# prismformore/Multi-Task-Transformer

Measured on NVIDIA H100. Metric: images/sec, higher is better.
Workload: dtype bf16x3 (split-bf16 operands, fp32 accumulate)

## Files before the change

### multi-task-transformer_b200/csrc/gemm_common.cuh

```cuda
#pragma once
#include "host_common.h"
#include "ptx.cuh"

namespace mtt {

constexpr int BM = 128;
constexpr int BK = 64;
constexpr int kEpiWarps = 8;
constexpr int kGemmThreads = 128 + kEpiWarps * 32;
constexpr uint32_t kTileBytes = BM * BK * 2;

struct GemmParams {
  int M, N;
  int num_kb, taps, ksize, dil, mode;
  int NB, H, W, TW, TH, tiles_x, tiles_y;
  int tiles_m;
  int tiles_n;
  int cin_pad;
  int k_last_steps;
  uint32_t a_box_bytes;
  const float* bias;
  int act;
  const float* residual;
  long long ldr;
  int res_row_mod;
  float* out_f32;
  long long ldo_f32;
  __nv_bfloat16* out_hi;
  __nv_bfloat16* out_lo;
  long long ldo_bf;
  int in_group, out_group, out_offset;
  int out_row_stride;
  int vec_ok;
  int a_groups_per_tile;
  int debug;
  int sk_tiles;
  float* sk_part;
  unsigned int* sk_flags;
};

constexpr size_t kSkFlagBytes = 16384;
constexpr size_t sk_workspace_bytes(int units) { return kSkFlagBytes + (size_t)units * BM * 256 * 4; }

constexpr int kMaxGroup = 32;
struct GroupProblem {
  const float* bias;
  const float* residual;
  float* out_f32;
  __nv_bfloat16* out_hi;
  __nv_bfloat16* out_lo;
};
struct GemmGroup {
  int count;
  int tiles_per_problem;
  GroupProblem prob[kMaxGroup];
};
struct GemmGroupMaps {
  CUtensorMap m[kMaxGroup][4];
};

int gemm_prepare(const mtt_gemm_desc* d, int b_box_rows, GemmParams& p, CUtensorMap maps[4]);

template <int NSPLIT>
__device__ __forceinline__ void load_a_tile(const GemmParams& p, const CUtensorMap* tmA_hi,
                                            const CUtensorMap* tmA_lo, uint8_t* sa, uint64_t* bar, int ms,
                                            int kb, int dy, int dx) {
  auto ld2 = [&](void* dst, const CUtensorMap* m, int c0, int c1) { tma_load_2d(dst, m, bar, c0, c1); };
  auto ld3 = [&](void* dst, const CUtensorMap* m, int c0, int c1, int c2) { tma_load_3d(dst, m, bar, c0, c1, c2); };
  auto ld4 = [&](void* dst, const CUtensorMap* m, int c0, int c1, int c2, int c3) {
    tma_load_4d(dst, m, bar, c0, c1, c2, c3);
  };
  if (p.mode == 0 && p.a_groups_per_tile > 0) {
    ld3(sa, tmA_hi, kb * BK, 0, ms * p.a_groups_per_tile);
    if (NSPLIT == 2) ld3(sa + kTileBytes, tmA_lo, kb * BK, 0, ms * p.a_groups_per_tile);
  } else if (p.mode == 0) {
    ld2(sa, tmA_hi, kb * BK, ms * BM);
    if (NSPLIT == 2) ld2(sa + kTileBytes, tmA_lo, kb * BK, ms * BM);
  } else {
    const int per_img = p.tiles_x * p.tiles_y;
    const int cb = ms / per_img;
    const int r = ms - cb * per_img;
    const int cy = (r / p.tiles_x) * p.TH + dy;
    const int cx = (r % p.tiles_x) * p.TW + dx;
    ld4(sa, tmA_hi, kb * BK, cx, cy, cb);
    if (NSPLIT == 2) ld4(sa + kTileBytes, tmA_lo, kb * BK, cx, cy, cb);
  }
}

struct RowInfo {
  long long mo;
  long long mr;
  bool ok;
};
__device__ __forceinline__ RowInfo row_info(const GemmParams& p, int ms, int row) {
  RowInfo r;
  long long m;
  if (p.mode == 0) {
    m = (long long)ms * BM + row;
    r.ok = m < p.M;
    if (p.a_groups_per_tile > 0) r.ok = r.ok && ms < p.tiles_m;
  } else {
    const int per_img = p.tiles_x * p.tiles_y;
    const int cb = ms / per_img;
    const int t = ms - cb * per_img;
    const int y = (t / p.tiles_x) * p.TH + row / p.TW;
    const int x = (t % p.tiles_x) * p.TW + row % p.TW;
    r.ok = (cb < p.NB) && (row < p.TW * p.TH) && (y < p.H) && (x < p.W);
    m = ((long long)cb * p.H + y) * p.W + x;
  }
  r.mo = m;
  if (p.in_group > 0) r.mo = (m / p.in_group) * p.out_group + p.out_offset + (m % p.in_group) * p.out_row_stride;
  r.mr = (p.res_row_mod > 0) ? (m % p.res_row_mod) : r.mo;
  return r;
}

enum { kOutF32 = 1, kOutSplit = 2, kOutBoth = 3 };

__device__ __forceinline__ float4 epilogue_bias4(const GemmParams& p, int n, bool full) {
  float4 b = make_float4(0.f, 0.f, 0.f, 0.f);
  if (!p.bias) return b;
  if (full) return __ldg(reinterpret_cast<const float4*>(p.bias + n));
  if (n < p.N) b.x = __ldg(p.bias + n);
  if (n + 1 < p.N) b.y = __ldg(p.bias + n + 1);
  if (n + 2 < p.N) b.z = __ldg(p.bias + n + 2);
  if (n + 3 < p.N) b.w = __ldg(p.bias + n + 3);
  return b;
}
template <int ACT>
__device__ __forceinline__ float epilogue_op(float v, float b, float r, bool bias, bool res) {
  if (bias) v += b;
  if (ACT == MTT_ACT_GELU) v = gelu_erf(v);
  if (ACT == MTT_ACT_RELU) v = fmaxf(v, 0.f);
  if (res) v += r;
  return v;
}
template <int ACT, int OUT>
__device__ __forceinline__ void epilogue_store4(const GemmParams& p, float4 v, float4 b, float4 r, long long of,
                                                long long ob, int n, bool full) {
  const bool bias = p.bias != nullptr, res = p.residual != nullptr;
  v.x = epilogue_op<ACT>(v.x, b.x, r.x, bias, res);
  v.y = epilogue_op<ACT>(v.y, b.y, r.y, bias, res);
  v.z = epilogue_op<ACT>(v.z, b.z, r.z, bias, res);
  v.w = epilogue_op<ACT>(v.w, b.w, r.w, bias, res);
  if (p.debug & 4) {
    asm volatile("" ::"f"(v.x), "f"(v.y), "f"(v.z), "f"(v.w));
    return;
  }
  if (full) {
    if (OUT & kOutF32) *reinterpret_cast<float4*>(p.out_f32 + of) = v;
    if (OUT & kOutSplit) {
      uint2 h, l;
      split_pack2(v.x, v.y, h.x, l.x);
      split_pack2(v.z, v.w, h.y, l.y);
      *reinterpret_cast<uint2*>(p.out_hi + ob) = h;
      if (p.out_lo) *reinterpret_cast<uint2*>(p.out_lo + ob) = l;
    }
    return;
  }
  const float e[4] = {v.x, v.y, v.z, v.w};
#pragma unroll
  for (int k = 0; k < 4; ++k) {
    if (n + k >= p.N) break;
    if (OUT & kOutF32) p.out_f32[of + k] = e[k];
    if (OUT & kOutSplit) {
      __nv_bfloat16 h, l;
      split_bf16(e[k], h, l);
      p.out_hi[ob + k] = h;
      if (p.out_lo) p.out_lo[ob + k] = l;
    }
  }
}

int launch_gemm_tiles(const mtt_gemm_desc* d, int bn, cudaStream_t stream);
int launch_gemm_tiles_grouped(const mtt_gemm_desc* d, int count, int bn, cudaStream_t stream);
void set_gemm_streamk(int mode);
int streamk_tiles(int tiles, int k_iters, int pairs);
int streamk_schedule_host(int tiles, int k_iters, int pairs, int pair, int* out, int max_pieces);

}
```

### multi-task-transformer_b200/csrc/gemm_host.cu

```cuda
#include <stdlib.h>

#include "gemm_common.cuh"

namespace mtt {

static void pick_conv_tile(int H, int W, int* TW, int* TH) {
  double best = -1;
  int btw = 1, bth = 1;
  for (int tw = 1; tw <= 128 && tw <= W; ++tw) {
    int th = 128 / tw;
    if (th > H) th = H;
    if (th < 1) continue;
    const long long tiles = (long long)((W + tw - 1) / tw) * ((H + th - 1) / th);
    const double eff = (double)H * W / ((double)tiles * 128.0);
    if (eff > best + 1e-9 || (eff > best - 1e-9 && tw > btw)) {
      best = eff;
      btw = tw;
      bth = th;
    }
  }
  *TW = btw;
  *TH = bth;
}

static int make_split_maps(const void* hi, const void* lo, int nsplit, int rank, const uint64_t* dims,
                           const uint64_t* strides, const uint32_t* box, CUtensorMap* maps) {
  int rc = make_tmap_bf16(&maps[0], hi, rank, dims, strides, box);
  if (rc) return rc;
  if (nsplit == 2) return make_tmap_bf16(&maps[1], lo, rank, dims, strides, box);
  maps[1] = maps[0];
  return MTT_OK;
}

int gemm_prepare(const mtt_gemm_desc* d, int b_box_rows, GemmParams& p, CUtensorMap maps[4]) {
  if (!d) return set_error(MTT_ERR_BAD_SHAPE, "mtt_gemm: null descriptor");
  if (d->M <= 0 || d->N <= 0 || d->K <= 0)
    return set_error(MTT_ERR_BAD_SHAPE, "mtt_gemm: M=%d N=%d K=%d must be positive", d->M, d->N, d->K);
  if (d->nsplit != 1 && d->nsplit != 2)
    return set_error(MTT_ERR_BAD_SHAPE, "mtt_gemm: nsplit=%d (1 or 2)", d->nsplit);
  if (!d->a_hi || !d->b_hi || (d->nsplit == 2 && (!d->a_lo || !d->b_lo)))
    return set_error(MTT_ERR_BAD_SHAPE, "mtt_gemm: missing operand plane");
  if (!d->out_f32 && !d->out_hi) return set_error(MTT_ERR_BAD_SHAPE, "mtt_gemm: no output");
  if (d->act != MTT_ACT_NONE && d->act != MTT_ACT_GELU && d->act != MTT_ACT_RELU)
    return set_error(MTT_ERR_BAD_SHAPE, "mtt_gemm: act=%d (0 none, 1 GELU, 2 ReLU)", d->act);
  if (d->lda % 8 || d->ldb % 8)
    return set_error(MTT_ERR_MISALIGNED, "mtt_gemm: lda=%lld ldb=%lld must be multiples of 8",
                     (long long)d->lda, (long long)d->ldb);

  p = GemmParams{};
  {
    static int dbg = -1;
    if (dbg < 0) {
      const char* e = getenv("MTT_GEMM_DEBUG");
      dbg = e ? atoi(e) : 0;
    }
    p.debug = dbg;
  }
  p.M = d->M;
  p.N = d->N;
  p.mode = d->mode;
  p.num_kb = (d->K + BK - 1) / BK;
  p.k_last_steps = (d->K - (p.num_kb - 1) * BK + 15) / 16;
  p.tiles_n = 0;
  p.bias = d->bias;
  p.act = d->act;
  p.residual = d->residual;
  p.ldr = d->ldr;
  p.res_row_mod = d->res_row_mod;
  p.out_f32 = d->out_f32;
  p.ldo_f32 = d->ldo_f32;
  p.out_hi = static_cast<__nv_bfloat16*>(d->out_hi);
  p.out_lo = static_cast<__nv_bfloat16*>(d->out_lo);
  p.ldo_bf = d->ldo_bf;
  p.in_group = d->in_group;
  p.out_group = d->out_group;
  p.out_offset = d->out_offset;
  p.out_row_stride = d->out_row_stride > 1 ? d->out_row_stride : 1;
  if (p.out_hi && d->nsplit == 2 && !p.out_lo)
    return set_error(MTT_ERR_BAD_SHAPE, "mtt_gemm: out_lo missing for nsplit=2");

  auto al16 = [](const void* q) { return (reinterpret_cast<uintptr_t>(q) & 15) == 0; };
  p.vec_ok = 1;
  if (d->bias && !al16(d->bias)) p.vec_ok = 0;
  if (d->residual && (!al16(d->residual) || d->ldr % 4)) p.vec_ok = 0;
  if (d->out_f32 && (!al16(d->out_f32) || d->ldo_f32 % 4)) p.vec_ok = 0;
  if (d->out_hi && (!al16(d->out_hi) || d->ldo_bf % 8 || (p.out_lo && !al16(p.out_lo)))) p.vec_ok = 0;

  int rc;
  const int ksq = (d->mode == 1) ? d->ksize * d->ksize : 1;
  if (d->mode == 0 && d->a_group_rows > 0) {
    const int g = d->a_group_rows;
    if (g > BM || d->M % g || d->a_group_stride < g)
      return set_error(MTT_ERR_BAD_SHAPE, "mtt_gemm: a_group_rows=%d must divide M=%d and be <= %d", g, d->M, BM);
    const int ngroups = d->M / g;
    const int gpt = BM / g;
    if (ngroups > gpt && BM % g)
      return set_error(MTT_ERR_BAD_SHAPE, "mtt_gemm: %d groups of %d rows need %d %% %d == 0", ngroups, g, BM, g);
    p.taps = 1;
    p.ksize = 1;
    p.dil = 1;
    p.cin_pad = 0;
    p.a_groups_per_tile = ngroups < gpt ? ngroups : gpt;
    p.tiles_m = (ngroups + p.a_groups_per_tile - 1) / p.a_groups_per_tile;
    if (p.tiles_m > 1 && p.a_groups_per_tile * g != BM)
      return set_error(MTT_ERR_BAD_SHAPE, "mtt_gemm: gathered A tiles must be full");
    p.a_box_bytes = (uint32_t)(p.a_groups_per_tile * g) * BK * 2;
    const uint64_t dims[3] = {(uint64_t)d->K, (uint64_t)g, (uint64_t)ngroups};
    const uint64_t str[2] = {(uint64_t)d->lda * 2, (uint64_t)d->a_group_stride * d->lda * 2};
    const uint32_t box[3] = {BK, (uint32_t)g, (uint32_t)p.a_groups_per_tile};
    if ((rc = make_split_maps(d->a_hi, d->a_lo, d->nsplit, 3, dims, str, box, &maps[0]))) return rc;
  } else if (d->mode == 0) {
    p.taps = 1;
    p.ksize = 1;
    p.dil = 1;
    p.cin_pad = 0;
    p.tiles_m = (d->M + BM - 1) / BM;
    p.a_box_bytes = kTileBytes;
    const uint64_t dims[2] = {(uint64_t)d->K, (uint64_t)d->M};
    const uint64_t str[1] = {(uint64_t)d->lda * 2};
    const uint32_t box[2] = {BK, BM};
    if ((rc = make_split_maps(d->a_hi, d->a_lo, d->nsplit, 2, dims, str, box, &maps[0]))) return rc;
  } else if (d->mode == 1) {
    if (d->B <= 0 || d->H <= 0 || d->W <= 0 || (long long)d->B * d->H * d->W != d->M)
      return set_error(MTT_ERR_BAD_SHAPE, "mtt_gemm(conv): B*H*W = %d*%d*%d != M = %d", d->B, d->H,
                       d->W, d->M);
    if (d->ksize != 1 && d->ksize != 3)
      return set_error(MTT_ERR_BAD_SHAPE, "mtt_gemm(conv): ksize=%d (1 or 3)", d->ksize);
    if (d->dil < 1) return set_error(MTT_ERR_BAD_SHAPE, "mtt_gemm(conv): dil=%d", d->dil);
    p.taps = ksq;
    p.ksize = d->ksize;
    p.dil = d->dil;
    p.cin_pad = p.num_kb * BK;
    p.NB = d->B;
    p.H = d->H;
    p.W = d->W;
    pick_conv_tile(d->H, d->W, &p.TW, &p.TH);
    p.tiles_x = (d->W + p.TW - 1) / p.TW;
    p.tiles_y = (d->H + p.TH - 1) / p.TH;
    p.tiles_m = d->B * p.tiles_x * p.tiles_y;
    p.a_box_bytes = (uint32_t)(p.TW * p.TH) * BK * 2;
    const uint64_t dims[4] = {(uint64_t)d->K, (uint64_t)d->W, (uint64_t)d->H, (uint64_t)d->B};
    const uint64_t str[3] = {(uint64_t)d->lda * 2, (uint64_t)d->W * d->lda * 2,
                             (uint64_t)d->H * d->W * d->lda * 2};
    const uint32_t box[4] = {BK, (uint32_t)p.TW, (uint32_t)p.TH, 1};
    if ((rc = make_split_maps(d->a_hi, d->a_lo, d->nsplit, 4, dims, str, box, &maps[0]))) return rc;
  } else {
    return set_error(MTT_ERR_BAD_SHAPE, "mtt_gemm: mode=%d", d->mode);
  }
  {
    const uint64_t ktot = (d->mode == 1) ? (uint64_t)ksq * p.cin_pad : (uint64_t)d->K;
    if ((uint64_t)d->ldb < ktot)
      return set_error(MTT_ERR_BAD_SHAPE, "mtt_gemm: ldb=%lld < packed K=%llu", (long long)d->ldb,
                       (unsigned long long)ktot);
    const uint64_t dims[2] = {ktot, (uint64_t)d->N};
    const uint64_t str[1] = {(uint64_t)d->ldb * 2};
    const uint32_t box[2] = {BK, (uint32_t)b_box_rows};
    if ((rc = make_split_maps(d->b_hi, d->b_lo, d->nsplit, 2, dims, str, box, &maps[2]))) return rc;
  }
  return MTT_OK;
}

static int g_variant = -1;

static int tile_width(const mtt_gemm_desc* d, int count) {
  static int grouped = -1;
  if (g_variant < 0) {
    const char* e = getenv("MTT_GEMM_VARIANT");
    g_variant = e ? atoi(e) : 0;
  }
  if (grouped < 0) {
    const char* e = getenv("MTT_GEMM_GROUPED_VARIANT");
    grouped = e ? atoi(e) : 0;
  }
  int v = g_variant;
  if (v == 0 && count > 1) v = grouped;
  if (v == 0) {
    const int n256 = (d->N + 255) / 256 * 256;
    const long long wide_tiles = (long long)count * ((d->M + 127) / 128) * (n256 / 256);
    if (count > 1) {
      v = (d->a_group_rows == 0 && d->M >= 512 && d->N >= 256 && (n256 - d->N) * 8 <= n256 && wide_tiles >= sm_count())
              ? 2 : 1;
    } else if (d->mode == 1) {
      const long long k_eff = (long long)d->K * d->ksize * d->ksize;
      v = (k_eff >= 2048 && wide_tiles >= sm_count() && d->N > 256 && (n256 - d->N) * 8 <= n256) ? 2 : 1;
    } else {
      const bool wide = d->N >= 512 && (n256 - d->N) * 8 <= n256;
      v = (wide && d->M > 128 && (d->N >= 2048 || d->K >= 2048)) ? 2 : 1;
    }
  }
  return v == 2 ? 256 : 128;
}

}

extern "C" void mtt_set_gemm_variant(int v) { mtt::g_variant = v; }
extern "C" void mtt_set_gemm_streamk(int mode) { mtt::set_gemm_streamk(mode); }
extern "C" int mtt_debug_streamk_schedule(int32_t tiles, int32_t k_iters, int32_t pairs, int32_t pair, int32_t* pieces,
                                          int32_t max_pieces) {
  return mtt::streamk_schedule_host(tiles, k_iters, pairs, pair, pieces, max_pieces);
}
extern "C" size_t mtt_gemm_streamk_bytes(void) {
  const int n = mtt::sm_count();
  return mtt::sk_workspace_bytes(n > 0 ? n : 132);
}

extern "C" int mtt_gemm(const mtt_gemm_desc* d, mtt_stream_t stream_) {
  using namespace mtt;
  cudaStream_t stream = static_cast<cudaStream_t>(stream_);
  if (!d) return set_error(MTT_ERR_BAD_SHAPE, "mtt_gemm: null descriptor");
  const int bn = tile_width(d, 1);
  const int taps = d->mode == 1 ? d->ksize * d->ksize : 1;
  ProfileScope prof(stream, 0, 2.0 * d->M * d->N * d->K * taps, d->M, d->N, d->K * taps);
  return launch_gemm_tiles(d, bn, stream);
}

extern "C" int mtt_gemm_grouped(const mtt_gemm_desc* d, int32_t count, mtt_stream_t stream_) {
  using namespace mtt;
  cudaStream_t stream = static_cast<cudaStream_t>(stream_);
  if (!d || count <= 0) return set_error(MTT_ERR_BAD_SHAPE, "mtt_gemm_grouped: no problems");
  if (count == 1) return mtt_gemm(d, stream_);
  if (count > kMaxGroup) return set_error(MTT_ERR_BAD_SHAPE, "mtt_gemm_grouped: %d problems > %d", count, kMaxGroup);
  const mtt_gemm_desc& a = d[0];
  for (int g = 1; g < count; ++g) {
    const mtt_gemm_desc& b = d[g];
    const bool same = a.M == b.M && a.N == b.N && a.K == b.K && a.nsplit == b.nsplit && a.mode == b.mode && a.B == b.B &&
                      a.H == b.H && a.W == b.W && a.ksize == b.ksize && a.dil == b.dil && a.act == b.act &&
                      a.lda == b.lda && a.ldb == b.ldb && a.ldr == b.ldr && a.res_row_mod == b.res_row_mod &&
                      a.ldo_f32 == b.ldo_f32 && a.ldo_bf == b.ldo_bf && a.in_group == b.in_group &&
                      a.out_group == b.out_group && a.out_offset == b.out_offset && a.out_row_stride == b.out_row_stride &&
                      a.a_group_rows == b.a_group_rows && a.a_group_stride == b.a_group_stride &&
                      (a.bias == nullptr) == (b.bias == nullptr) && (a.residual == nullptr) == (b.residual == nullptr) &&
                      (a.out_f32 == nullptr) == (b.out_f32 == nullptr) && (a.out_hi == nullptr) == (b.out_hi == nullptr);
    if (!same)
      return set_error(MTT_ERR_BAD_SHAPE, "mtt_gemm_grouped: problem %d differs from problem 0 in more than its pointers", g);
  }
  double fl = 0;
  for (int g = 0; g < count; ++g) fl += 2.0 * d[g].M * d[g].N * d[g].K * (d[g].mode == 1 ? d[g].ksize * d[g].ksize : 1);
  ProfileScope prof(stream, 0, fl, a.M * count, a.N, a.K * (a.mode == 1 ? a.ksize * a.ksize : 1));
  return launch_gemm_tiles_grouped(d, count, tile_width(d, count), stream);
}
```

### multi-task-transformer_b200/csrc/gemm_tc.cu

```cuda
#include <stdlib.h>

#include <type_traits>

#include "gemm_common.cuh"

namespace mtt {

constexpr int kEpiCols = 32;

template <int NSPLIT, int BN>
struct GemmCfg {
  static constexpr int kNsplit = NSPLIT, kBN = BN;
  static constexpr uint32_t kBTileBytes = BN * BK * 2;
  static constexpr uint32_t kStageBytes = NSPLIT * (kTileBytes + kBTileBytes);
  static constexpr int kStages = (200 * 1024) / kStageBytes;
  static constexpr uint32_t kEpiBufBytes = kEpiWarps * 2 * 16 * kEpiCols * 4;
  static constexpr uint32_t kRowMapBytes = kEpiWarps * 16 * 8;
  static constexpr uint32_t kSmemBytes = kStages * kStageBytes + 256 + kEpiBufBytes + kRowMapBytes + 1024;
  static_assert(kSmemBytes <= 227 * 1024, "exceeds the per-block shared memory of sm_90");
  static constexpr int kRegPlanes = BN == 128 ? NSPLIT : 1;
};

struct SkSched {
  int n_sk;
  int tile0, k0_0, k1_0;
  int k1_1;
  int dp_first, dp_step;
  int n_seg;
  long long W;
};
template <bool SK>
__host__ __device__ __forceinline__ SkSched sk_schedule(const GemmParams& p, int pair, int num_pairs, int num_tiles, int k_iters) {
  SkSched s;
  s.n_sk = 0;
  s.tile0 = s.k0_0 = s.k1_0 = s.k1_1 = 0;
  s.W = 0;
  s.dp_first = pair;
  s.dp_step = num_pairs;
  if (SK && p.sk_tiles > 0) {
    s.W = (long long)p.sk_tiles * k_iters;
    const long long b = (long long)pair * s.W / num_pairs, e = (long long)(pair + 1) * s.W / num_pairs;
    if (e > b) {
      const int t0 = (int)(b / k_iters);
      const long long t0_end = (long long)(t0 + 1) * k_iters;
      s.tile0 = t0;
      s.k0_0 = (int)(b - (long long)t0 * k_iters);
      s.k1_0 = (int)((e < t0_end ? e : t0_end) - (long long)t0 * k_iters);
      s.n_sk = 1;
      if (e > t0_end) {
        s.k1_1 = (int)(e - t0_end);
        s.n_sk = 2;
      }
    }
    s.dp_first = p.sk_tiles + pair;
  }
  const int left = num_tiles - s.dp_first;
  s.n_seg = s.n_sk + (left > 0 ? (left + s.dp_step - 1) / s.dp_step : 0);
  return s;
}
__host__ __device__ __forceinline__ void sk_piece(const SkSched& s, int si, int k_iters, int& tile, int& k0, int& k1) {
  if (si < s.n_sk) {
    tile = s.tile0 + si;
    k0 = si == 0 ? s.k0_0 : 0;
    k1 = si == 0 ? s.k1_0 : s.k1_1;
  } else {
    tile = s.dp_first + (si - s.n_sk) * s.dp_step;
    k0 = 0;
    k1 = k_iters;
  }
}
__device__ __forceinline__ void sk_flag_publish(unsigned int* f) {
  asm volatile("st.release.gpu.global.u32 [%0], %1;" ::"l"(f), "r"(1u) : "memory");
}
__device__ __forceinline__ unsigned int sk_flag_peek(const unsigned int* f) {
  unsigned int v;
  asm volatile("ld.acquire.gpu.global.u32 %0, [%1];" : "=r"(v) : "l"(f) : "memory");
  return v;
}


constexpr uint32_t kTurnBar = 1;

struct PieceCoords {
  int g, mt, nt;
};
template <bool GROUPED>
__device__ __forceinline__ PieceCoords piece_coords(const GemmParams& p, int tpp, int tile) {
  const int g = GROUPED ? tile / tpp : 0;
  const int tl = GROUPED ? tile - g * tpp : tile;
  return PieceCoords{g, tl % p.tiles_m, tl / p.tiles_m};
}

template <int NSPLIT, int BN, bool GROUPED>
__device__ __forceinline__ void produce(const CUtensorMap (*maps)[4], const GemmParams& p, const SkSched& sched,
                                        int tpp, int k_iters, uint8_t* smem, uint64_t* full_bar, uint64_t* empty_bar) {
  using Cfg = GemmCfg<NSPLIT, BN>;
  int stage = 0;
  uint32_t phase = 0;
  const uint32_t stage_tx = NSPLIT * (p.a_box_bytes + Cfg::kBTileBytes);
  for (int si = 0; si < sched.n_seg; ++si) {
    int tile, kbeg, kend;
    sk_piece(sched, si, k_iters, tile, kbeg, kend);
    const PieceCoords pc = piece_coords<GROUPED>(p, tpp, tile);
    const CUtensorMap* tmA_hi = &maps[pc.g][0];
    const CUtensorMap* tmA_lo = &maps[pc.g][1];
    const CUtensorMap* tmB_hi = &maps[pc.g][2];
    const CUtensorMap* tmB_lo = &maps[pc.g][3];
    for (int ki = kbeg; ki < kend; ++ki) {
      const int tap = ki / p.num_kb, kb = ki - tap * p.num_kb;
      const int dy = (tap / p.ksize - p.ksize / 2) * p.dil;
      const int dx = (tap % p.ksize - p.ksize / 2) * p.dil;
      mbar_wait(&empty_bar[stage], phase ^ 1);
      uint8_t* sa = smem + stage * Cfg::kStageBytes;
      uint8_t* sb = sa + NSPLIT * kTileBytes;
      if (elect_one()) {
        if (p.debug & 1) {
          mbar_arrive(&full_bar[stage]);
        } else {
          mbar_arrive_expect_tx(&full_bar[stage], stage_tx);
          load_a_tile<NSPLIT>(p, tmA_hi, tmA_lo, sa, &full_bar[stage], pc.mt, kb, dy, dx);
          const int kcoord = tap * p.cin_pad + kb * BK;
          tma_load_2d(sb, tmB_hi, &full_bar[stage], kcoord, pc.nt * BN);
          if (NSPLIT == 2) tma_load_2d(sb + Cfg::kBTileBytes, tmB_lo, &full_bar[stage], kcoord, pc.nt * BN);
        }
      }
      __syncwarp();
      if (++stage == Cfg::kStages) {
        stage = 0;
        phase ^= 1;
      }
    }
  }
}

struct ConsumerWarp {
  int lane;
  int cw;
  int ew;
  int row0, col0;
  int wrow0;
  uint32_t a_off;
  uint32_t a_frag_off;
  int a_chunk, a_xor;
  uint32_t ebuf, rbuf, rmap;
};
template <typename Cfg>
__device__ __forceinline__ ConsumerWarp consumer_warp(uint8_t* smem, int warp, int lane) {
  ConsumerWarp c;
  c.lane = lane;
  c.cw = (warp - 4) >> 2;
  c.ew = warp - 4;
  c.row0 = c.cw * 64 + (warp & 3) * 16 + (lane >> 2);
  c.col0 = 2 * (lane & 3);
  c.a_off = (uint32_t)c.cw * 64 * 128;
  const int lrow = (warp & 3) * 16 + (lane & 7) + ((lane >> 3) & 1) * 8;
  c.a_frag_off = c.a_off + (uint32_t)lrow * 128;
  c.a_chunk = lane >> 4;
  c.a_xor = lane & 7;
  c.wrow0 = c.cw * 64 + (warp & 3) * 16;
  c.ebuf = smem_u32(smem + Cfg::kStages * Cfg::kStageBytes + 256) + c.ew * (2 * 16 * kEpiCols * 4);
  c.rbuf = c.ebuf + 16 * kEpiCols * 4;
  c.rmap = smem_u32(smem + Cfg::kStages * Cfg::kStageBytes + 256 + Cfg::kEpiBufBytes) + c.ew * 16 * 8;
  return c;
}

__device__ __forceinline__ void res_issue(const GemmParams& p, const ConsumerWarp& c, const float* res, int n0,
                                          int half) {
  const int n = n0 + 4 * (c.lane & 7);
#pragma unroll
  for (int k = 0; k < 2; ++k) {
    const int r = 8 * half + (c.lane >> 3) + 4 * k;
    const long long m = ld_shared_s64(c.rmap + 8 * r);
    const uint32_t dst = c.rbuf + (r * kEpiCols + 4 * (c.lane & 7)) * 4;
    const float* src = res + (m >= 0 ? m * p.ldr + n : 0);
    if (p.vec_ok) {
      const int cols = m >= 0 ? min(max(p.N - n, 0), 4) : 0;
      cp_async_cg16(dst, cols ? src : res, 4 * cols);
    } else {
#pragma unroll
      for (int e = 0; e < 4; ++e) {
        const bool in = m >= 0 && n + e < p.N;
        cp_async_ca4(dst + 4 * e, in ? src + e : res, in ? 4 : 0);
      }
    }
  }
  cp_async_commit();
}

template <int BN>
__device__ __forceinline__ void res_prefetch(const GemmParams& p, const ConsumerWarp& c, const float* res, int mt,
                                             int nt) {
  if (c.lane < 16) {
    const RowInfo ri = row_info(p, mt, c.wrow0 + c.lane);
    st_shared_s64(c.rmap + 8 * c.lane, ri.ok ? ri.mr : -1);
  }
  __syncwarp();
  res_issue(p, c, res, nt * BN, 0);
  res_issue(p, c, res, nt * BN, 1);
}

__device__ __forceinline__ void wait_turn(int cw) {
  if (cw == 0) bar_sync<kTurnBar, 256>(); else bar_sync<kTurnBar + 1, 256>();
}
__device__ __forceinline__ void pass_turn(int cw) {
  if (cw == 0) bar_arrive<kTurnBar + 1, 256>(); else bar_arrive<kTurnBar, 256>();
}

template <int NSPLIT, int BN>
__device__ __forceinline__ void mma_piece(const GemmParams& p, const ConsumerWarp& c, uint8_t* smem, uint64_t* full_bar,
                                          uint64_t* empty_bar, int kbeg, int kend, int& stage, uint32_t& phase,
                                          float (&acc)[BN / 2], float (&part)[64],
                                          uint32_t (&afr)[BK / 16][GemmCfg<NSPLIT, BN>::kRegPlanes][4]) {
  using Cfg = GemmCfg<NSPLIT, BN>;
  constexpr int kRegPlanes = Cfg::kRegPlanes;
#pragma unroll
  for (int i = 0; i < BN / 2; ++i) acc[i] = 0.f;
  int kb = kbeg % p.num_kb;
  for (int ki = kbeg; ki < kend; ++ki) {
    const int nks = (++kb == p.num_kb) ? p.k_last_steps : BK / 16;
    if (kb == p.num_kb) kb = 0;
    mbar_wait(&full_bar[stage], phase);
    const uint32_t sa = smem_u32(smem + stage * Cfg::kStageBytes);
    const uint32_t a_lo = sa + kTileBytes + c.a_off;
    const uint32_t b_hi = sa + NSPLIT * kTileBytes, b_lo = b_hi + Cfg::kBTileBytes;
    {
      const uint32_t fa = sa + c.a_frag_off;
#pragma unroll
      for (int ks = 0; ks < BK / 16; ++ks) {
        const uint32_t sw = (uint32_t)(((2 * ks + c.a_chunk) ^ c.a_xor) << 4);
#pragma unroll
        for (int s = 0; s < kRegPlanes; ++s) ldmatrix_x4(afr[ks][s], fa + s * kTileBytes + sw);
      }
    }
#pragma unroll
    for (int hn = 0; hn < BN / 128; ++hn) {
      const uint32_t bo = (uint32_t)hn * 128 * 128;
      wait_turn(c.cw);
      wgmma_fence_regs(part);
      wgmma_fence();
#pragma unroll
      for (int ks = 0; ks < BK / 16; ++ks) {
        if (ks >= nks) break;
        const uint64_t bdh = gmma_desc_sw128(b_hi + bo + ks * 32);
        wgmma_rs_n128<0>(part, afr[ks][0], bdh, ks > 0 ? 1 : 0);
        if (NSPLIT == 2) {
          wgmma_rs_n128<0>(part, afr[ks][0], gmma_desc_sw128(b_lo + bo + ks * 32), 1);
          if (kRegPlanes == 2)
            wgmma_rs_n128<0>(part, afr[ks][1], bdh, 1);
          else
            wgmma_ss_n128<0>(part, gmma_desc_sw128(a_lo + ks * 32), bdh, 1);
        }
      }
      wgmma_commit();
      pass_turn(c.cw);
      wgmma_wait<0>();
      wgmma_fence_regs(part);
#pragma unroll
      for (int ks = 0; ks < BK / 16; ++ks)
#pragma unroll
        for (int s = 0; s < kRegPlanes; ++s) wgmma_fence_regs(afr[ks][s]);
#pragma unroll
      for (int i = 0; i < 64; ++i) acc[hn * 64 + i] += part[i];
    }
    __syncwarp();
    if (c.lane == 0) mbar_arrive(&empty_bar[stage]);
    if (++stage == Cfg::kStages) {
      stage = 0;
      phase ^= 1;
    }
  }
}

template <int BN>
__device__ __forceinline__ void sk_contribute(const GemmParams& p, const ConsumerWarp& c, const float (&acc)[BN / 2]) {
  float* part = p.sk_part + (size_t)blockIdx.x * BM * 256;
#pragma unroll
  for (int i = 0; i < BN / 8; ++i) {
#pragma unroll
    for (int h = 0; h < 2; ++h)
      *reinterpret_cast<float2*>(part + (size_t)(c.row0 + 8 * h) * 256 + 8 * i + c.col0) =
          make_float2(acc[4 * i + 2 * h], acc[4 * i + 2 * h + 1]);
  }
  __threadfence();
  __syncwarp();
  if (c.lane == 0) sk_flag_publish(p.sk_flags + blockIdx.x * kEpiWarps + c.ew);
}

template <int BN>
__device__ __forceinline__ void sk_collect(const GemmParams& p, const ConsumerWarp& c, const SkSched& sched, int tile,
                                           int k_iters, float (&acc)[BN / 2]) {
  const long long tile_kend = (long long)(tile + 1) * k_iters;
  for (int pp = blockIdx.x + 1; pp < (int)gridDim.x && (long long)pp * sched.W / gridDim.x < tile_kend; ++pp) {
    unsigned int* flag = p.sk_flags + pp * kEpiWarps + c.ew;
    if (c.lane == 0) {
      while (sk_flag_peek(flag) == 0) {
      }
    }
    __syncwarp();
    __threadfence();
    const float* part = p.sk_part + (size_t)pp * BM * 256;
#pragma unroll
    for (int i = 0; i < BN / 8; ++i) {
#pragma unroll
      for (int h = 0; h < 2; ++h) {
        const float2 a = __ldcg(reinterpret_cast<const float2*>(part + (size_t)(c.row0 + 8 * h) * 256 + 8 * i + c.col0));
        acc[4 * i + 2 * h] += a.x;
        acc[4 * i + 2 * h + 1] += a.y;
      }
    }
    __syncwarp();
    if (c.lane == 0) *reinterpret_cast<volatile unsigned int*>(flag) = 0u;
  }
}

__device__ __forceinline__ GemmParams problem_params(const GemmParams& p, const GemmGroup* grp, int g) {
  GemmParams pg = p;
  const GroupProblem& gp = grp->prob[g];
  pg.bias = gp.bias;
  pg.residual = gp.residual;
  pg.out_f32 = gp.out_f32;
  pg.out_hi = gp.out_hi;
  pg.out_lo = gp.out_lo;
  return pg;
}

template <int BN, int ACT, int OUT>
__device__ __forceinline__ void epilogue_piece(const GemmParams& p, const GemmParams& pq, const ConsumerWarp& cs,
                                               const float (&acc)[BN / 2], int mt, int nt) {
  const int lane = cs.lane;
  const int lr = lane >> 3, c4 = 4 * (lane & 7);
  long long of_map, ob_map;
  int rows_ok = 0;
  {
    const RowInfo ri = row_info(p, mt, cs.wrow0 + (lane & 15));
    of_map = ri.mo * pq.ldo_f32;
    ob_map = ri.mo * pq.ldo_bf;
#pragma unroll
    for (int q = 0; q < 4; ++q) rows_ok |= (__shfl_sync(0xffffffffu, (int)ri.ok, 4 * q + lr) & 1) << q;
  }
  const uint32_t e_wr = cs.ebuf + ((lane >> 2) * kEpiCols + cs.col0) * 4, e_sw = ((lane >> 2) & 3) * 32;
  const uint32_t e_rd = cs.ebuf + (lr * kEpiCols + (c4 ^ (lr << 3))) * 4;
  const uint32_t r_rd = cs.rbuf + (lr * kEpiCols + c4) * 4;
  constexpr int kChunks = BN / kEpiCols;
#pragma unroll 1
  for (int c = 0; c < kChunks; ++c) {
    const int n0 = nt * BN + c * kEpiCols, n = n0 + c4;
    const bool full = pq.vec_ok && n + 4 <= pq.N;
    const float4 b = epilogue_bias4(pq, n, full);
#pragma unroll
    for (int cc = 0; cc < kChunks; ++cc) {
      if (cc != c) continue;
#pragma unroll
      for (int j = 0; j < kEpiCols / 8; ++j)
#pragma unroll
        for (int h = 0; h < 2; ++h) {
          const int i = cc * (kEpiCols / 8) + j;
          st_shared_v2(e_wr + h * 8 * kEpiCols * 4 + ((j * 32) ^ e_sw), acc[4 * i + 2 * h], acc[4 * i + 2 * h + 1]);
        }
    }
    auto store_rows = [&](int half) {
#pragma unroll 1
      for (int q = 2 * half; q < 2 * half + 2; ++q) {
        const float4 v = ld_shared_v4(e_rd + q * 4 * kEpiCols * 4);
        const float4 rv = pq.residual ? ld_shared_v4(r_rd + q * 4 * kEpiCols * 4) : make_float4(0.f, 0.f, 0.f, 0.f);
        const long long of = (OUT & kOutF32) ? __shfl_sync(0xffffffffu, of_map, 4 * q + lr) + n : 0;
        const long long ob = (OUT & kOutSplit) ? __shfl_sync(0xffffffffu, ob_map, 4 * q + lr) + n : 0;
        if (rows_ok & (1 << q)) epilogue_store4<ACT, OUT>(pq, v, b, rv, of, ob, n, full);
      }
    };
    if (pq.residual) cp_async_wait<1>();
    __syncwarp();
    store_rows(0);
    if (pq.residual) {
      __syncwarp();
      if (c + 1 < kChunks) {
        res_issue(p, cs, pq.residual, n0 + kEpiCols, 0);
        cp_async_wait<1>();
      } else {
        cp_async_wait<0>();
      }
      __syncwarp();
    }
    store_rows(1);
    __syncwarp();
    if (pq.residual && c + 1 < kChunks) res_issue(p, cs, pq.residual, n0 + kEpiCols, 1);
  }
}

template <int NSPLIT, int BN, bool GROUPED, bool SK, int ACT, int OUT>
__device__ __forceinline__ void gemm_tc_body(const CUtensorMap (*maps)[4], const GemmParams& p, const GemmGroup* grp) {
  static_assert(!SK || (BN == 256 && !GROUPED), "stream-K: single-problem kernel with 256-wide tiles only");
  using Cfg = GemmCfg<NSPLIT, BN>;
  constexpr int ST = Cfg::kStages;
  extern __shared__ uint8_t smem_raw[];
  uint8_t* smem = reinterpret_cast<uint8_t*>((reinterpret_cast<uintptr_t>(smem_raw) + 1023) &
                                             ~static_cast<uintptr_t>(1023));
  uint64_t* full_bar = reinterpret_cast<uint64_t*>(smem + ST * Cfg::kStageBytes);
  uint64_t* empty_bar = full_bar + ST;

  const int warp = threadIdx.x >> 5;
  const int tpp = p.tiles_m * p.tiles_n;
  const int num_tiles = GROUPED ? tpp * grp->count : tpp;
  const int k_iters = p.taps * p.num_kb;
  const SkSched sched = sk_schedule<SK>(p, blockIdx.x, gridDim.x, num_tiles, k_iters);

  if (threadIdx.x == 0) {
    tma_prefetch_desc(&maps[0][0]);
    tma_prefetch_desc(&maps[0][2]);
    if (NSPLIT == 2) {
      tma_prefetch_desc(&maps[0][1]);
      tma_prefetch_desc(&maps[0][3]);
    }
    for (int s = 0; s < ST; ++s) {
      mbar_init(&full_bar[s], 1);
      mbar_init(&empty_bar[s], kEpiWarps);
    }
    fence_barrier_init();
  }
  __syncthreads();

  if (warp < 4) {
    setmaxnreg_dec<40>();
    if (warp == 0) produce<NSPLIT, BN, GROUPED>(maps, p, sched, tpp, k_iters, smem, full_bar, empty_bar);
  } else {
    setmaxnreg_inc<232>();
    const ConsumerWarp c = consumer_warp<Cfg>(smem, warp, threadIdx.x & 31);
    int stage = 0;
    uint32_t phase = 0;
    float acc[BN / 2];
    float part[64];
    uint32_t afr[BK / 16][Cfg::kRegPlanes][4];
    if (c.cw == 1) pass_turn(c.cw);
    for (int si = 0; si < sched.n_seg; ++si) {
      int tile, kbeg, kend;
      sk_piece(sched, si, k_iters, tile, kbeg, kend);
      const PieceCoords pc = piece_coords<GROUPED>(p, tpp, tile);
      const float* res = GROUPED ? grp->prob[pc.g].residual : p.residual;
      if (res && !(SK && kbeg > 0) && !(p.debug & 2))
        res_prefetch<BN>(p, c, res, pc.mt, pc.nt);
      mma_piece<NSPLIT, BN>(p, c, smem, full_bar, empty_bar, kbeg, kend, stage, phase, acc, part, afr);
      const bool sk_contrib = SK && kbeg > 0;
      const bool sk_owner = SK && kbeg == 0 && kend < k_iters;
      if (SK && sk_contrib) {
        sk_contribute<BN>(p, c, acc);
        continue;
      }
      if (SK && sk_owner) sk_collect<BN>(p, c, sched, tile, k_iters, acc);
      if (p.debug & 2) continue;
      if constexpr (GROUPED)
        epilogue_piece<BN, ACT, OUT>(p, problem_params(p, grp, pc.g), c, acc, pc.mt, pc.nt);
      else
        epilogue_piece<BN, ACT, OUT>(p, p, c, acc, pc.mt, pc.nt);
    }
    if (c.cw == 0) wait_turn(c.cw);
  }
}

struct GemmMaps1 {
  CUtensorMap m[1][4];
};

template <int NSPLIT, int BN, bool SK, int ACT, int OUT>
__global__ void __launch_bounds__(kGemmThreads, 1)
gemm_tc_kernel(const __grid_constant__ GemmMaps1 maps, const GemmParams p) {
  gemm_tc_body<NSPLIT, BN, false, SK, ACT, OUT>(maps.m, p, nullptr);
}

template <int NSPLIT, int BN, int ACT, int OUT>
__global__ void __launch_bounds__(kGemmThreads, 1)
gemm_tc_grouped_kernel(const __grid_constant__ GemmGroupMaps maps, const __grid_constant__ GemmGroup grp,
                       const GemmParams p) {
  gemm_tc_body<NSPLIT, BN, true, false, ACT, OUT>(maps.m, p, &grp);
}

template <typename Cfg, typename Kernel, typename... Args>
static int launch_kernel(Kernel kernel, bool (&done)[kMaxDevices], const char* what, int grid, cudaStream_t stream,
                         const Args&... args) {
  const int dev_ = current_device();
  if (!done[dev_]) {
    cudaError_t e = cudaFuncSetAttribute(kernel, cudaFuncAttributeMaxDynamicSharedMemorySize, Cfg::kSmemBytes);
    if (e != cudaSuccess) return set_error(MTT_ERR_LAUNCH, "%s: cudaFuncSetAttribute: %s", what, cudaGetErrorString(e));
    done[dev_] = true;
  }
  kernel<<<grid, kGemmThreads, Cfg::kSmemBytes, stream>>>(args...);
  return check_launch(what);
}

template <int ACT_, int OUT_>
struct EpiKind {
  static constexpr int ACT = ACT_, OUT = OUT_;
};
template <int ACT, typename F>
static int with_epilogue_out(const GemmParams& p, F&& f) {
  if (!p.out_hi) return f(EpiKind<ACT, kOutF32>{});
  if (!p.out_f32) return f(EpiKind<ACT, kOutSplit>{});
  return f(EpiKind<ACT, kOutBoth>{});
}
template <typename F>
static int with_epilogue(const GemmParams& p, F&& f) {
  switch (p.act) {
    case MTT_ACT_NONE: return with_epilogue_out<MTT_ACT_NONE>(p, f);
    case MTT_ACT_GELU: return with_epilogue_out<MTT_ACT_GELU>(p, f);
    case MTT_ACT_RELU: return with_epilogue_out<MTT_ACT_RELU>(p, f);
  }
  return set_error(MTT_ERR_BAD_SHAPE, "mtt_gemm: no kernel for act=%d", p.act);
}

template <typename F>
static int with_tile(int nsplit, int bn, F&& f) {
  if (bn == 256) return nsplit == 2 ? f(GemmCfg<2, 256>{}) : f(GemmCfg<1, 256>{});
  return nsplit == 2 ? f(GemmCfg<2, 128>{}) : f(GemmCfg<1, 128>{});
}

template <typename Maps>
static int launch_gemm(const Maps& maps, const GemmGroup* grp, const GemmParams& p, int nsplit, int bn, int grid,
                       cudaStream_t stream) {
  constexpr bool kGrouped = std::is_same<Maps, GemmGroupMaps>::value;
  const bool sk = p.sk_tiles > 0;
  const char* what = kGrouped ? "mtt_gemm_grouped" : sk ? "mtt_gemm(stream-K)" : "mtt_gemm";
  return with_tile(nsplit, bn, [&](auto cfg) {
    using Cfg = decltype(cfg);
    return with_epilogue(p, [&](auto e) {
      constexpr int NSPLIT = Cfg::kNsplit, BN = Cfg::kBN, ACT = decltype(e)::ACT, OUT = decltype(e)::OUT;
      static bool done[2][kMaxDevices] = {};
      if constexpr (kGrouped) {
        return launch_kernel<Cfg>(gemm_tc_grouped_kernel<NSPLIT, BN, ACT, OUT>, done[0], what, grid, stream, maps, *grp,
                                  p);
      } else {
        if constexpr (BN == 256)
          if (sk)
            return launch_kernel<Cfg>(gemm_tc_kernel<NSPLIT, BN, true, ACT, OUT>, done[1], what, grid, stream, maps, p);
        return launch_kernel<Cfg>(gemm_tc_kernel<NSPLIT, BN, false, ACT, OUT>, done[0], what, grid, stream, maps, p);
      }
    });
  });
}

int launch_gemm_tiles_grouped(const mtt_gemm_desc* d, int count, int bn, cudaStream_t stream) {
  GemmParams p;
  GemmGroupMaps gm;
  GemmGroup grp;
  grp.count = count;
  for (int g = 0; g < count; ++g) {
    GemmParams pg;
    int rc = gemm_prepare(&d[g], bn, pg, gm.m[g]);
    if (rc) return rc;
    pg.tiles_n = (d[g].N + bn - 1) / bn;
    if (g == 0) {
      p = pg;
    } else {
      p.vec_ok = p.vec_ok && pg.vec_ok;
    }
    grp.prob[g] = GroupProblem{pg.bias, pg.residual, pg.out_f32, pg.out_hi, pg.out_lo};
  }
  grp.tiles_per_problem = p.tiles_m * p.tiles_n;
  const int tiles = grp.tiles_per_problem * grp.count;
  return launch_gemm(gm, &grp, p, d[0].nsplit, bn, tiles < sm_count() ? tiles : sm_count(), stream);
}

static int g_streamk = -1;
void set_gemm_streamk(int mode) { g_streamk = mode < 0 ? 0 : (mode > 2 ? 2 : mode); }

int streamk_tiles(int tiles, int k_iters, int pairs) {
  if (g_streamk < 0) {
    const char* e = getenv("MTT_GEMM_STREAMK");
    set_gemm_streamk(e ? atoi(e) : 1);
  }
  if (!g_streamk || pairs < 2 || pairs * 2 * kEpiWarps * 4 > (int)kSkFlagBytes) return 0;
  const int r = tiles % pairs;
  if (r == 0 || (pairs - r) * 16 < pairs || (long long)r * k_iters / pairs < 4) return 0;
  if (g_streamk == 1 && (tiles >= pairs || (pairs - r) * 2 < pairs || k_iters < 32)) return 0;
  return r;
}

int streamk_schedule_host(int tiles, int k_iters, int pairs, int pair, int* out, int max_pieces) {
  GemmParams p = {};
  p.sk_tiles = streamk_tiles(tiles, k_iters, pairs);
  const int num_pairs = p.sk_tiles > 0 ? pairs : (tiles < pairs ? tiles : pairs);
  if (pair >= num_pairs) return 0;
  const SkSched s = sk_schedule<true>(p, pair, num_pairs, tiles, k_iters);
  int n = 0;
  for (int si = 0; si < s.n_seg && n < max_pieces; ++si, ++n) sk_piece(s, si, k_iters, out[3 * n], out[3 * n + 1], out[3 * n + 2]);
  return s.n_seg;
}

int launch_gemm_tiles(const mtt_gemm_desc* d, int bn, cudaStream_t stream) {
  GemmParams p;
  GemmMaps1 gm;
  int rc = gemm_prepare(d, bn, p, gm.m[0]);
  if (rc) return rc;
  p.tiles_n = (d->N + bn - 1) / bn;
  const int tiles = p.tiles_m * p.tiles_n;
  const int units = sm_count();
  if (bn == 256 && d->sk_ws) {
    const int r = streamk_tiles(tiles, p.taps * p.num_kb, units);
    if (r > 0) {
      if ((size_t)d->sk_ws_bytes < sk_workspace_bytes(units) || (reinterpret_cast<uintptr_t>(d->sk_ws) & 255))
        return set_error(MTT_ERR_BAD_SHAPE, "mtt_gemm: sk_ws of %lld bytes (256-byte aligned) < required %zu "
                         "(mtt_gemm_streamk_bytes)", (long long)d->sk_ws_bytes, sk_workspace_bytes(units));
      p.sk_tiles = r;
      p.sk_flags = static_cast<unsigned int*>(d->sk_ws);
      p.sk_part = reinterpret_cast<float*>(static_cast<uint8_t*>(d->sk_ws) + kSkFlagBytes);
    }
  }
  const int grid = p.sk_tiles > 0 ? units : (tiles < units ? tiles : units);
  return launch_gemm(gm, nullptr, p, d->nsplit, bn, grid, stream);
}

}
```

### multi-task-transformer_b200/csrc/ptx.cuh

```cuda
#pragma once
#include <cuda.h>
#include <cuda_bf16.h>
#include <cuda_runtime.h>
#include <stdint.h>

namespace mtt {

__device__ __forceinline__ uint32_t smem_u32(const void* p) {
  return static_cast<uint32_t>(__cvta_generic_to_shared(p));
}

__device__ __forceinline__ bool elect_one() {
  uint32_t pred = 0;
  asm volatile(
      "{\n\t"
      ".reg .pred P;\n\t"
      "elect.sync _|P, 0xffffffff;\n\t"
      "selp.b32 %0, 1, 0, P;\n\t"
      "}\n"
      : "=r"(pred));
  return pred != 0;
}

template <uint32_t kRegs>
__device__ __forceinline__ void setmaxnreg_dec() {
  asm volatile("setmaxnreg.dec.sync.aligned.u32 %0;" ::"n"(kRegs));
}
template <uint32_t kRegs>
__device__ __forceinline__ void setmaxnreg_inc() {
  asm volatile("setmaxnreg.inc.sync.aligned.u32 %0;" ::"n"(kRegs));
}

template <uint32_t kId, uint32_t kCount>
__device__ __forceinline__ void bar_sync() {
  asm volatile("bar.sync %0, %1;" ::"n"(kId), "n"(kCount) : "memory");
}
template <uint32_t kId, uint32_t kCount>
__device__ __forceinline__ void bar_arrive() {
  asm volatile("bar.arrive %0, %1;" ::"n"(kId), "n"(kCount) : "memory");
}

__device__ __forceinline__ unsigned int clock32() {
  unsigned int c;
  asm volatile("mov.u32 %0, %%clock;" : "=r"(c));
  return c;
}
__device__ __forceinline__ unsigned int smid() {
  unsigned int c;
  asm volatile("mov.u32 %0, %%smid;" : "=r"(c));
  return c;
}

__device__ __forceinline__ void mbar_init(uint64_t* bar, uint32_t count) {
  asm volatile("mbarrier.init.shared::cta.b64 [%0], %1;" ::"r"(smem_u32(bar)), "r"(count));
}
__device__ __forceinline__ void fence_barrier_init() {
  asm volatile("fence.mbarrier_init.release.cluster;" ::: "memory");
}
__device__ __forceinline__ void fence_proxy_async() {
  asm volatile("fence.proxy.async.shared::cta;" ::: "memory");
}
__device__ __forceinline__ void mbar_arrive_expect_tx(uint64_t* bar, uint32_t bytes) {
  asm volatile("mbarrier.arrive.expect_tx.shared::cta.b64 _, [%0], %1;" ::"r"(smem_u32(bar)),
               "r"(bytes)
               : "memory");
}
__device__ __forceinline__ void mbar_arrive(uint64_t* bar) {
  asm volatile("mbarrier.arrive.shared::cta.b64 _, [%0];" ::"r"(smem_u32(bar)) : "memory");
}
__device__ __forceinline__ bool mbar_try_wait(uint64_t* bar, uint32_t parity) {
  uint32_t ok;
  asm volatile(
      "{\n\t"
      ".reg .pred p;\n\t"
      "mbarrier.try_wait.parity.shared::cta.b64 p, [%1], %2;\n\t"
      "selp.b32 %0, 1, 0, p;\n\t"
      "}\n"
      : "=r"(ok)
      : "r"(smem_u32(bar)), "r"(parity)
      : "memory");
  return ok != 0;
}
__device__ __forceinline__ void mbar_wait(uint64_t* bar, uint32_t parity) {
  while (!mbar_try_wait(bar, parity)) {
  }
}

__device__ __forceinline__ void tma_prefetch_desc(const CUtensorMap* m) {
  asm volatile("prefetch.tensormap [%0];" ::"l"(reinterpret_cast<uint64_t>(m)) : "memory");
}
__device__ __forceinline__ void tma_load_2d(void* smem, const CUtensorMap* m, uint64_t* bar, int c0,
                                            int c1) {
  asm volatile(
      "cp.async.bulk.tensor.2d.shared::cluster.global.mbarrier::complete_tx::bytes [%0], [%1, {%3, "
      "%4}], [%2];" ::"r"(smem_u32(smem)),
      "l"(reinterpret_cast<uint64_t>(m)), "r"(smem_u32(bar)), "r"(c0), "r"(c1)
      : "memory");
}
__device__ __forceinline__ void tma_load_3d(void* smem, const CUtensorMap* m, uint64_t* bar, int c0,
                                            int c1, int c2) {
  asm volatile(
      "cp.async.bulk.tensor.3d.shared::cluster.global.mbarrier::complete_tx::bytes [%0], [%1, {%3, "
      "%4, %5}], [%2];" ::"r"(smem_u32(smem)),
      "l"(reinterpret_cast<uint64_t>(m)), "r"(smem_u32(bar)), "r"(c0), "r"(c1), "r"(c2)
      : "memory");
}
__device__ __forceinline__ void tma_load_4d(void* smem, const CUtensorMap* m, uint64_t* bar, int c0,
                                            int c1, int c2, int c3) {
  asm volatile(
      "cp.async.bulk.tensor.4d.shared::cluster.global.mbarrier::complete_tx::bytes [%0], [%1, {%3, "
      "%4, %5, %6}], [%2];" ::"r"(smem_u32(smem)),
      "l"(reinterpret_cast<uint64_t>(m)), "r"(smem_u32(bar)), "r"(c0), "r"(c1), "r"(c2), "r"(c3)
      : "memory");
}

__device__ __forceinline__ void tma_store_3d(const CUtensorMap* m, const void* smem, int c0, int c1, int c2) {
  asm volatile("cp.async.bulk.tensor.3d.global.shared::cta.bulk_group [%0, {%2, %3, %4}], [%1];" ::"l"(
                   reinterpret_cast<uint64_t>(m)),
               "r"(smem_u32(smem)), "r"(c0), "r"(c1), "r"(c2)
               : "memory");
}
__device__ __forceinline__ void tma_store_commit() { asm volatile("cp.async.bulk.commit_group;" ::: "memory"); }
__device__ __forceinline__ void tma_store_wait_read() { asm volatile("cp.async.bulk.wait_group.read 0;" ::: "memory"); }
__device__ __forceinline__ void tma_store_wait_all() { asm volatile("cp.async.bulk.wait_group 0;" ::: "memory"); }

__device__ __forceinline__ void cp_async_cg16(uint32_t dst, const void* src, uint32_t src_bytes) {
  asm volatile("cp.async.cg.shared.global [%0], [%1], 16, %2;" ::"r"(dst), "l"(src), "r"(src_bytes) : "memory");
}
__device__ __forceinline__ void cp_async_ca4(uint32_t dst, const void* src, uint32_t src_bytes) {
  asm volatile("cp.async.ca.shared.global [%0], [%1], 4, %2;" ::"r"(dst), "l"(src), "r"(src_bytes) : "memory");
}
__device__ __forceinline__ void cp_async_commit() { asm volatile("cp.async.commit_group;" ::: "memory"); }

__device__ __forceinline__ void st_shared_v2(uint32_t a, float x, float y) {
  asm volatile("st.shared.v2.f32 [%0], {%1, %2};" ::"r"(a), "f"(x), "f"(y) : "memory");
}
__device__ __forceinline__ float4 ld_shared_v4(uint32_t a) {
  float4 v;
  asm volatile("ld.shared.v4.f32 {%0, %1, %2, %3}, [%4];" : "=f"(v.x), "=f"(v.y), "=f"(v.z), "=f"(v.w) : "r"(a));
  return v;
}
__device__ __forceinline__ void st_shared_s64(uint32_t a, long long v) {
  asm volatile("st.shared.s64 [%0], %1;" ::"r"(a), "l"(v) : "memory");
}
__device__ __forceinline__ long long ld_shared_s64(uint32_t a) {
  long long v;
  asm volatile("ld.shared.s64 %0, [%1];" : "=l"(v) : "r"(a));
  return v;
}
template <int kPending>
__device__ __forceinline__ void cp_async_wait() {
  asm volatile("cp.async.wait_group %0;" ::"n"(kPending) : "memory");
}

__device__ __forceinline__ void tma_prefetch_2d(const CUtensorMap* m, int c0, int c1) {
  asm volatile("cp.async.bulk.prefetch.tensor.2d.L2.global [%0, {%1, %2}];" ::"l"(reinterpret_cast<uint64_t>(m)),
               "r"(c0), "r"(c1)
               : "memory");
}
__device__ __forceinline__ void tma_prefetch_3d(const CUtensorMap* m, int c0, int c1, int c2) {
  asm volatile("cp.async.bulk.prefetch.tensor.3d.L2.global [%0, {%1, %2, %3}];" ::"l"(
                   reinterpret_cast<uint64_t>(m)),
               "r"(c0), "r"(c1), "r"(c2)
               : "memory");
}
__device__ __forceinline__ void tma_prefetch_4d(const CUtensorMap* m, int c0, int c1, int c2, int c3) {
  asm volatile("cp.async.bulk.prefetch.tensor.4d.L2.global [%0, {%1, %2, %3, %4}];" ::"l"(
                   reinterpret_cast<uint64_t>(m)),
               "r"(c0), "r"(c1), "r"(c2), "r"(c3)
               : "memory");
}

__device__ __forceinline__ void wgmma_fence() { asm volatile("wgmma.fence.sync.aligned;" ::: "memory"); }
__device__ __forceinline__ void wgmma_commit() { asm volatile("wgmma.commit_group.sync.aligned;" ::: "memory"); }
template <int kPending>
__device__ __forceinline__ void wgmma_wait() {
  asm volatile("wgmma.wait_group.sync.aligned %0;" ::"n"(kPending) : "memory");
}
template <int kN>
__device__ __forceinline__ void wgmma_fence_regs(float (&d)[kN]) {
#pragma unroll
  for (int i = 0; i < kN; ++i) asm volatile("" : "+f"(d[i])::"memory");
}

__device__ __forceinline__ uint64_t gmma_desc_sw128(uint32_t smem_addr) {
  uint64_t d = 0;
  d |= (uint64_t)((smem_addr & 0x3FFFF) >> 4);
  d |= (uint64_t)1 << 16;
  d |= (uint64_t)(1024 >> 4) << 32;
  d |= (uint64_t)1 << 62;
  return d;
}

template <int kTransB>
__device__ __forceinline__ void wgmma_ss_n64(float (&d)[32], uint64_t adesc, uint64_t bdesc, int scale_d) {
  asm volatile(
      "{\n\t.reg .pred p;\n\tsetp.ne.b32 p, %34, 0;\n\t"
      "wgmma.mma_async.sync.aligned.m64n64k16.f32.bf16.bf16 {%0, %1, %2, %3, %4, %5, %6, %7, %8, %9, %10, %11, %12, %13, %14, %15, %16, %17, %18, %19, %20, %21, %22, %23, %24, %25, %26, %27, %28, %29, %30, %31}, %32, %33, p, 1, 1, 0, %35;\n\t}\n"
      : "+f"(d[0]), "+f"(d[1]), "+f"(d[2]), "+f"(d[3]), "+f"(d[4]), "+f"(d[5]), "+f"(d[6]), "+f"(d[7]), "+f"(d[8]), "+f"(d[9]), "+f"(d[10]), "+f"(d[11]), "+f"(d[12]), "+f"(d[13]), "+f"(d[14]), "+f"(d[15]), "+f"(d[16]), "+f"(d[17]), "+f"(d[18]), "+f"(d[19]), "+f"(d[20]), "+f"(d[21]), "+f"(d[22]), "+f"(d[23]), "+f"(d[24]), "+f"(d[25]), "+f"(d[26]), "+f"(d[27]), "+f"(d[28]), "+f"(d[29]), "+f"(d[30]), "+f"(d[31])
      : "l"(adesc), "l"(bdesc), "r"(scale_d), "n"(kTransB));
}

template <int kTransB>
__device__ __forceinline__ void wgmma_ss_n128(float (&d)[64], uint64_t adesc, uint64_t bdesc, int scale_d) {
  asm volatile(
      "{\n\t.reg .pred p;\n\tsetp.ne.b32 p, %66, 0;\n\t"
      "wgmma.mma_async.sync.aligned.m64n128k16.f32.bf16.bf16 {%0, %1, %2, %3, %4, %5, %6, %7, %8, %9, %10, %11, %12, %13, %14, %15, %16, %17, %18, %19, %20, %21, %22, %23, %24, %25, %26, %27, %28, %29, %30, %31, %32, %33, %34, %35, %36, %37, %38, %39, %40, %41, %42, %43, %44, %45, %46, %47, %48, %49, %50, %51, %52, %53, %54, %55, %56, %57, %58, %59, %60, %61, %62, %63}, %64, %65, p, 1, 1, 0, %67;\n\t}\n"
      : "+f"(d[0]), "+f"(d[1]), "+f"(d[2]), "+f"(d[3]), "+f"(d[4]), "+f"(d[5]), "+f"(d[6]), "+f"(d[7]), "+f"(d[8]), "+f"(d[9]), "+f"(d[10]), "+f"(d[11]), "+f"(d[12]), "+f"(d[13]), "+f"(d[14]), "+f"(d[15]), "+f"(d[16]), "+f"(d[17]), "+f"(d[18]), "+f"(d[19]), "+f"(d[20]), "+f"(d[21]), "+f"(d[22]), "+f"(d[23]), "+f"(d[24]), "+f"(d[25]), "+f"(d[26]), "+f"(d[27]), "+f"(d[28]), "+f"(d[29]), "+f"(d[30]), "+f"(d[31]), "+f"(d[32]), "+f"(d[33]), "+f"(d[34]), "+f"(d[35]), "+f"(d[36]), "+f"(d[37]), "+f"(d[38]), "+f"(d[39]), "+f"(d[40]), "+f"(d[41]), "+f"(d[42]), "+f"(d[43]), "+f"(d[44]), "+f"(d[45]), "+f"(d[46]), "+f"(d[47]), "+f"(d[48]), "+f"(d[49]), "+f"(d[50]), "+f"(d[51]), "+f"(d[52]), "+f"(d[53]), "+f"(d[54]), "+f"(d[55]), "+f"(d[56]), "+f"(d[57]), "+f"(d[58]), "+f"(d[59]), "+f"(d[60]), "+f"(d[61]), "+f"(d[62]), "+f"(d[63])
      : "l"(adesc), "l"(bdesc), "r"(scale_d), "n"(kTransB));
}

template <int kTransB>
__device__ __forceinline__ void wgmma_ss_n256(float (&d)[128], uint64_t adesc, uint64_t bdesc, int scale_d) {
  asm volatile(
      "{\n\t.reg .pred p;\n\tsetp.ne.b32 p, %130, 0;\n\t"
      "wgmma.mma_async.sync.aligned.m64n256k16.f32.bf16.bf16 {%0, %1, %2, %3, %4, %5, %6, %7, %8, %9, %10, %11, %12, %13, %14, %15, %16, %17, %18, %19, %20, %21, %22, %23, %24, %25, %26, %27, %28, %29, %30, %31, %32, %33, %34, %35, %36, %37, %38, %39, %40, %41, %42, %43, %44, %45, %46, %47, %48, %49, %50, %51, %52, %53, %54, %55, %56, %57, %58, %59, %60, %61, %62, %63, %64, %65, %66, %67, %68, %69, %70, %71, %72, %73, %74, %75, %76, %77, %78, %79, %80, %81, %82, %83, %84, %85, %86, %87, %88, %89, %90, %91, %92, %93, %94, %95, %96, %97, %98, %99, %100, %101, %102, %103, %104, %105, %106, %107, %108, %109, %110, %111, %112, %113, %114, %115, %116, %117, %118, %119, %120, %121, %122, %123, %124, %125, %126, %127}, %128, %129, p, 1, 1, 0, %131;\n\t}\n"
      : "+f"(d[0]), "+f"(d[1]), "+f"(d[2]), "+f"(d[3]), "+f"(d[4]), "+f"(d[5]), "+f"(d[6]), "+f"(d[7]), "+f"(d[8]), "+f"(d[9]), "+f"(d[10]), "+f"(d[11]), "+f"(d[12]), "+f"(d[13]), "+f"(d[14]), "+f"(d[15]), "+f"(d[16]), "+f"(d[17]), "+f"(d[18]), "+f"(d[19]), "+f"(d[20]), "+f"(d[21]), "+f"(d[22]), "+f"(d[23]), "+f"(d[24]), "+f"(d[25]), "+f"(d[26]), "+f"(d[27]), "+f"(d[28]), "+f"(d[29]), "+f"(d[30]), "+f"(d[31]), "+f"(d[32]), "+f"(d[33]), "+f"(d[34]), "+f"(d[35]), "+f"(d[36]), "+f"(d[37]), "+f"(d[38]), "+f"(d[39]), "+f"(d[40]), "+f"(d[41]), "+f"(d[42]), "+f"(d[43]), "+f"(d[44]), "+f"(d[45]), "+f"(d[46]), "+f"(d[47]), "+f"(d[48]), "+f"(d[49]), "+f"(d[50]), "+f"(d[51]), "+f"(d[52]), "+f"(d[53]), "+f"(d[54]), "+f"(d[55]), "+f"(d[56]), "+f"(d[57]), "+f"(d[58]), "+f"(d[59]), "+f"(d[60]), "+f"(d[61]), "+f"(d[62]), "+f"(d[63]), "+f"(d[64]), "+f"(d[65]), "+f"(d[66]), "+f"(d[67]), "+f"(d[68]), "+f"(d[69]), "+f"(d[70]), "+f"(d[71]), "+f"(d[72]), "+f"(d[73]), "+f"(d[74]), "+f"(d[75]), "+f"(d[76]), "+f"(d[77]), "+f"(d[78]), "+f"(d[79]), "+f"(d[80]), "+f"(d[81]), "+f"(d[82]), "+f"(d[83]), "+f"(d[84]), "+f"(d[85]), "+f"(d[86]), "+f"(d[87]), "+f"(d[88]), "+f"(d[89]), "+f"(d[90]), "+f"(d[91]), "+f"(d[92]), "+f"(d[93]), "+f"(d[94]), "+f"(d[95]), "+f"(d[96]), "+f"(d[97]), "+f"(d[98]), "+f"(d[99]), "+f"(d[100]), "+f"(d[101]), "+f"(d[102]), "+f"(d[103]), "+f"(d[104]), "+f"(d[105]), "+f"(d[106]), "+f"(d[107]), "+f"(d[108]), "+f"(d[109]), "+f"(d[110]), "+f"(d[111]), "+f"(d[112]), "+f"(d[113]), "+f"(d[114]), "+f"(d[115]), "+f"(d[116]), "+f"(d[117]), "+f"(d[118]), "+f"(d[119]), "+f"(d[120]), "+f"(d[121]), "+f"(d[122]), "+f"(d[123]), "+f"(d[124]), "+f"(d[125]), "+f"(d[126]), "+f"(d[127])
      : "l"(adesc), "l"(bdesc), "r"(scale_d), "n"(kTransB));
}

template <int kTransB>
__device__ __forceinline__ void wgmma_rs_n64(float (&d)[32], const uint32_t (&a)[4], uint64_t bdesc, int scale_d) {
  asm volatile(
      "{\n\t.reg .pred p;\n\tsetp.ne.b32 p, %37, 0;\n\t"
      "wgmma.mma_async.sync.aligned.m64n64k16.f32.bf16.bf16 {%0, %1, %2, %3, %4, %5, %6, %7, %8, %9, %10, %11, %12, %13, %14, %15, %16, %17, %18, %19, %20, %21, %22, %23, %24, %25, %26, %27, %28, %29, %30, %31}, {%32, %33, %34, %35}, %36, p, 1, 1, %38;\n\t}\n"
      : "+f"(d[0]), "+f"(d[1]), "+f"(d[2]), "+f"(d[3]), "+f"(d[4]), "+f"(d[5]), "+f"(d[6]), "+f"(d[7]), "+f"(d[8]), "+f"(d[9]), "+f"(d[10]), "+f"(d[11]), "+f"(d[12]), "+f"(d[13]), "+f"(d[14]), "+f"(d[15]), "+f"(d[16]), "+f"(d[17]), "+f"(d[18]), "+f"(d[19]), "+f"(d[20]), "+f"(d[21]), "+f"(d[22]), "+f"(d[23]), "+f"(d[24]), "+f"(d[25]), "+f"(d[26]), "+f"(d[27]), "+f"(d[28]), "+f"(d[29]), "+f"(d[30]), "+f"(d[31])
      : "r"(a[0]), "r"(a[1]), "r"(a[2]), "r"(a[3]), "l"(bdesc), "r"(scale_d), "n"(kTransB));
}

template <int kTransB>
__device__ __forceinline__ void wgmma_rs_n128(float (&d)[64], const uint32_t (&a)[4], uint64_t bdesc, int scale_d) {
  asm volatile(
      "{\n\t.reg .pred p;\n\tsetp.ne.b32 p, %69, 0;\n\t"
      "wgmma.mma_async.sync.aligned.m64n128k16.f32.bf16.bf16 {%0, %1, %2, %3, %4, %5, %6, %7, %8, %9, %10, %11, %12, %13, %14, %15, %16, %17, %18, %19, %20, %21, %22, %23, %24, %25, %26, %27, %28, %29, %30, %31, %32, %33, %34, %35, %36, %37, %38, %39, %40, %41, %42, %43, %44, %45, %46, %47, %48, %49, %50, %51, %52, %53, %54, %55, %56, %57, %58, %59, %60, %61, %62, %63}, {%64, %65, %66, %67}, %68, p, 1, 1, %70;\n\t}\n"
      : "+f"(d[0]), "+f"(d[1]), "+f"(d[2]), "+f"(d[3]), "+f"(d[4]), "+f"(d[5]), "+f"(d[6]), "+f"(d[7]), "+f"(d[8]), "+f"(d[9]), "+f"(d[10]), "+f"(d[11]), "+f"(d[12]), "+f"(d[13]), "+f"(d[14]), "+f"(d[15]), "+f"(d[16]), "+f"(d[17]), "+f"(d[18]), "+f"(d[19]), "+f"(d[20]), "+f"(d[21]), "+f"(d[22]), "+f"(d[23]), "+f"(d[24]), "+f"(d[25]), "+f"(d[26]), "+f"(d[27]), "+f"(d[28]), "+f"(d[29]), "+f"(d[30]), "+f"(d[31]), "+f"(d[32]), "+f"(d[33]), "+f"(d[34]), "+f"(d[35]), "+f"(d[36]), "+f"(d[37]), "+f"(d[38]), "+f"(d[39]), "+f"(d[40]), "+f"(d[41]), "+f"(d[42]), "+f"(d[43]), "+f"(d[44]), "+f"(d[45]), "+f"(d[46]), "+f"(d[47]), "+f"(d[48]), "+f"(d[49]), "+f"(d[50]), "+f"(d[51]), "+f"(d[52]), "+f"(d[53]), "+f"(d[54]), "+f"(d[55]), "+f"(d[56]), "+f"(d[57]), "+f"(d[58]), "+f"(d[59]), "+f"(d[60]), "+f"(d[61]), "+f"(d[62]), "+f"(d[63])
      : "r"(a[0]), "r"(a[1]), "r"(a[2]), "r"(a[3]), "l"(bdesc), "r"(scale_d), "n"(kTransB));
}
template <int kN>
__device__ __forceinline__ void wgmma_fence_regs(uint32_t (&a)[kN]) {
#pragma unroll
  for (int i = 0; i < kN; ++i) asm volatile("" : "+r"(a[i])::"memory");
}

__device__ __forceinline__ void ldmatrix_x4(uint32_t (&r)[4], uint32_t smem_addr) {
  asm volatile("ldmatrix.sync.aligned.m8n8.x4.shared.b16 {%0, %1, %2, %3}, [%4];"
               : "=r"(r[0]), "=r"(r[1]), "=r"(r[2]), "=r"(r[3])
               : "r"(smem_addr)
               : "memory");
}


__device__ __forceinline__ void split_bf16(float x, __nv_bfloat16& hi, __nv_bfloat16& lo) {
  hi = __float2bfloat16_rn(x);
  lo = __float2bfloat16_rn(x - __bfloat162float(hi));
}
__device__ __forceinline__ uint32_t pack_bf16x2(float a, float b) {
  uint32_t r;
  asm("cvt.rn.bf16x2.f32 %0, %1, %2;" : "=r"(r) : "f"(b), "f"(a));
  return r;
}
__device__ __forceinline__ float bf16lo_to_f32(uint32_t packed) {
  return __uint_as_float(packed << 16);
}
__device__ __forceinline__ float bf16hi_to_f32(uint32_t packed) {
  return __uint_as_float(packed & 0xFFFF0000u);
}
__device__ __forceinline__ void split_pack2(float a, float b, uint32_t& hi, uint32_t& lo) {
  hi = pack_bf16x2(a, b);
  lo = pack_bf16x2(a - bf16lo_to_f32(hi), b - bf16hi_to_f32(hi));
}

__device__ __forceinline__ void split_pack2_alu(float a, float b, uint32_t& hi, uint32_t& lo) {
  const uint32_t ua = __float_as_uint(a) + 0x8000u, ub = __float_as_uint(b) + 0x8000u;
  hi = __byte_perm(ua, ub, 0x7632);
  const float ra = a - __uint_as_float(ua & 0xFFFF0000u), rb = b - __uint_as_float(ub & 0xFFFF0000u);
  lo = __byte_perm(__float_as_uint(ra) + 0x8000u, __float_as_uint(rb) + 0x8000u, 0x7632);
}

__device__ __forceinline__ float2 ffma2(float2 a, float2 b, float2 c) {
  return make_float2(fmaf(a.x, b.x, c.x), fmaf(a.y, b.y, c.y));
}

__device__ __forceinline__ float ex2_approx(float x) {
  float y;
  asm("ex2.approx.ftz.f32 %0, %1;" : "=f"(y) : "f"(x));
  return y;
}

__device__ __forceinline__ float gelu_erf(float x) {
  return 0.5f * x * (1.0f + erff(x * 0.70710678118654752440f));
}

}
```

Before: 171.9.

## Add 176-wide N tile GEMM variant with ring pipeline for better wave quantization

Adds a BN=176 tile configuration that uses m64n88k16 wgmma instructions (two halves per consumer). The host picks it when 176-wide tiles pad N less than 128-wide tiles and need fewer total tile-columns per wave across the SMs. The kernel body moves into a shared header, and the 176 path gets its own producer and MMA loops using a separate ring scheme. The aim is to cut padded N work and tail-wave waste. In exchange it adds kernel instantiations, more accumulator registers and a new untested pipeline path.

```diff
diff --git a/multi-task-transformer_b200/csrc/gemm_common.cuh b/multi-task-transformer_b200/csrc/gemm_common.cuh
--- a/multi-task-transformer_b200/csrc/gemm_common.cuh
+++ b/multi-task-transformer_b200/csrc/gemm_common.cuh
@@ -57,6 +57,9 @@
 };
 struct GemmGroupMaps {
   CUtensorMap m[kMaxGroup][4];
+};
+struct GemmMaps1 {
+  CUtensorMap m[1][4];
 };
 
 int gemm_prepare(const mtt_gemm_desc* d, int b_box_rows, GemmParams& p, CUtensorMap maps[4]);
@@ -173,6 +176,9 @@
 
 int launch_gemm_tiles(const mtt_gemm_desc* d, int bn, cudaStream_t stream);
 int launch_gemm_tiles_grouped(const mtt_gemm_desc* d, int count, int bn, cudaStream_t stream);
+template <typename Maps>
+int launch_gemm_176(const Maps& maps, const GemmGroup* grp, const GemmParams& p, int nsplit, int grid,
+                    cudaStream_t stream);
 void set_gemm_streamk(int mode);
 int streamk_tiles(int tiles, int k_iters, int pairs);
 int streamk_schedule_host(int tiles, int k_iters, int pairs, int pair, int* out, int max_pieces);
diff --git a/multi-task-transformer_b200/csrc/gemm_host.cu b/multi-task-transformer_b200/csrc/gemm_host.cu
--- a/multi-task-transformer_b200/csrc/gemm_host.cu
+++ b/multi-task-transformer_b200/csrc/gemm_host.cu
@@ -187,8 +187,14 @@
       const bool wide = d->N >= 512 && (n256 - d->N) * 8 <= n256;
       v = (wide && d->M > 128 && (d->N >= 2048 || d->K >= 2048)) ? 2 : 1;
     }
-  }
-  return v == 2 ? 256 : 128;
+    if (v == 1 && (d->N + 175) / 176 * 176 < (d->N + 127) / 128 * 128) {
+      const long long mt = (long long)count * ((d->M + 127) / 128), sms = sm_count() > 0 ? sm_count() : 1;
+      const long long waves128 = (mt * ((d->N + 127) / 128) + sms - 1) / sms;
+      const long long waves176 = (mt * ((d->N + 175) / 176) + sms - 1) / sms;
+      if (waves176 * 176 < waves128 * 128) v = 4;
+    }
+  }
+  return v == 2 ? 256 : v == 4 ? 176 : 128;
 }
 
 }
diff --git a/multi-task-transformer_b200/csrc/gemm_tc.cu b/multi-task-transformer_b200/csrc/gemm_tc.cu
--- a/multi-task-transformer_b200/csrc/gemm_tc.cu
+++ b/multi-task-transformer_b200/csrc/gemm_tc.cu
@@ -1,539 +1,20 @@
 #include <stdlib.h>
 
-#include <type_traits>
-
-#include "gemm_common.cuh"
+#include "gemm_tc_body.cuh"
 
 namespace mtt {
 
-constexpr int kEpiCols = 32;
-
-template <int NSPLIT, int BN>
-struct GemmCfg {
-  static constexpr int kNsplit = NSPLIT, kBN = BN;
-  static constexpr uint32_t kBTileBytes = BN * BK * 2;
-  static constexpr uint32_t kStageBytes = NSPLIT * (kTileBytes + kBTileBytes);
-  static constexpr int kStages = (200 * 1024) / kStageBytes;
-  static constexpr uint32_t kEpiBufBytes = kEpiWarps * 2 * 16 * kEpiCols * 4;
-  static constexpr uint32_t kRowMapBytes = kEpiWarps * 16 * 8;
-  static constexpr uint32_t kSmemBytes = kStages * kStageBytes + 256 + kEpiBufBytes + kRowMapBytes + 1024;
-  static_assert(kSmemBytes <= 227 * 1024, "exceeds the per-block shared memory of sm_90");
-  static constexpr int kRegPlanes = BN == 128 ? NSPLIT : 1;
-};
-
-struct SkSched {
-  int n_sk;
-  int tile0, k0_0, k1_0;
-  int k1_1;
-  int dp_first, dp_step;
-  int n_seg;
-  long long W;
-};
-template <bool SK>
-__host__ __device__ __forceinline__ SkSched sk_schedule(const GemmParams& p, int pair, int num_pairs, int num_tiles, int k_iters) {
-  SkSched s;
-  s.n_sk = 0;
-  s.tile0 = s.k0_0 = s.k1_0 = s.k1_1 = 0;
-  s.W = 0;
-  s.dp_first = pair;
-  s.dp_step = num_pairs;
-  if (SK && p.sk_tiles > 0) {
-    s.W = (long long)p.sk_tiles * k_iters;
-    const long long b = (long long)pair * s.W / num_pairs, e = (long long)(pair + 1) * s.W / num_pairs;
-    if (e > b) {
-      const int t0 = (int)(b / k_iters);
-      const long long t0_end = (long long)(t0 + 1) * k_iters;
-      s.tile0 = t0;
-      s.k0_0 = (int)(b - (long long)t0 * k_iters);
-      s.k1_0 = (int)((e < t0_end ? e : t0_end) - (long long)t0 * k_iters);
-      s.n_sk = 1;
-      if (e > t0_end) {
-        s.k1_1 = (int)(e - t0_end);
-        s.n_sk = 2;
-      }
-    }
-    s.dp_first = p.sk_tiles + pair;
-  }
-  const int left = num_tiles - s.dp_first;
-  s.n_seg = s.n_sk + (left > 0 ? (left + s.dp_step - 1) / s.dp_step : 0);
-  return s;
-}
-__host__ __device__ __forceinline__ void sk_piece(const SkSched& s, int si, int k_iters, int& tile, int& k0, int& k1) {
-  if (si < s.n_sk) {
-    tile = s.tile0 + si;
-    k0 = si == 0 ? s.k0_0 : 0;
-    k1 = si == 0 ? s.k1_0 : s.k1_1;
-  } else {
-    tile = s.dp_first + (si - s.n_sk) * s.dp_step;
-    k0 = 0;
-    k1 = k_iters;
-  }
-}
-__device__ __forceinline__ void sk_flag_publish(unsigned int* f) {
-  asm volatile("st.release.gpu.global.u32 [%0], %1;" ::"l"(f), "r"(1u) : "memory");
-}
-__device__ __forceinline__ unsigned int sk_flag_peek(const unsigned int* f) {
-  unsigned int v;
-  asm volatile("ld.acquire.gpu.global.u32 %0, [%1];" : "=r"(v) : "l"(f) : "memory");
-  return v;
-}
-
-
-constexpr uint32_t kTurnBar = 1;
-
-struct PieceCoords {
-  int g, mt, nt;
-};
-template <bool GROUPED>
-__device__ __forceinline__ PieceCoords piece_coords(const GemmParams& p, int tpp, int tile) {
-  const int g = GROUPED ? tile / tpp : 0;
-  const int tl = GROUPED ? tile - g * tpp : tile;
-  return PieceCoords{g, tl % p.tiles_m, tl / p.tiles_m};
-}
-
-template <int NSPLIT, int BN, bool GROUPED>
-__device__ __forceinline__ void produce(const CUtensorMap (*maps)[4], const GemmParams& p, const SkSched& sched,
-                                        int tpp, int k_iters, uint8_t* smem, uint64_t* full_bar, uint64_t* empty_bar) {
-  using Cfg = GemmCfg<NSPLIT, BN>;
-  int stage = 0;
-  uint32_t phase = 0;
-  const uint32_t stage_tx = NSPLIT * (p.a_box_bytes + Cfg::kBTileBytes);
-  for (int si = 0; si < sched.n_seg; ++si) {
-    int tile, kbeg, kend;
-    sk_piece(sched, si, k_iters, tile, kbeg, kend);
-    const PieceCoords pc = piece_coords<GROUPED>(p, tpp, tile);
-    const CUtensorMap* tmA_hi = &maps[pc.g][0];
-    const CUtensorMap* tmA_lo = &maps[pc.g][1];
-    const CUtensorMap* tmB_hi = &maps[pc.g][2];
-    const CUtensorMap* tmB_lo = &maps[pc.g][3];
-    for (int ki = kbeg; ki < kend; ++ki) {
-      const int tap = ki / p.num_kb, kb = ki - tap * p.num_kb;
-      const int dy = (tap / p.ksize - p.ksize / 2) * p.dil;
-      const int dx = (tap % p.ksize - p.ksize / 2) * p.dil;
-      mbar_wait(&empty_bar[stage], phase ^ 1);
-      uint8_t* sa = smem + stage * Cfg::kStageBytes;
-      uint8_t* sb = sa + NSPLIT * kTileBytes;
-      if (elect_one()) {
-        if (p.debug & 1) {
-          mbar_arrive(&full_bar[stage]);
-        } else {
-          mbar_arrive_expect_tx(&full_bar[stage], stage_tx);
-          load_a_tile<NSPLIT>(p, tmA_hi, tmA_lo, sa, &full_bar[stage], pc.mt, kb, dy, dx);
-          const int kcoord = tap * p.cin_pad + kb * BK;
-          tma_load_2d(sb, tmB_hi, &full_bar[stage], kcoord, pc.nt * BN);
-          if (NSPLIT == 2) tma_load_2d(sb + Cfg::kBTileBytes, tmB_lo, &full_bar[stage], kcoord, pc.nt * BN);
-        }
-      }
-      __syncwarp();
-      if (++stage == Cfg::kStages) {
-        stage = 0;
-        phase ^= 1;
-      }
-    }
-  }
-}
-
-struct ConsumerWarp {
-  int lane;
-  int cw;
-  int ew;
-  int row0, col0;
-  int wrow0;
-  uint32_t a_off;
-  uint32_t a_frag_off;
-  int a_chunk, a_xor;
-  uint32_t ebuf, rbuf, rmap;
-};
-template <typename Cfg>
-__device__ __forceinline__ ConsumerWarp consumer_warp(uint8_t* smem, int warp, int lane) {
-  ConsumerWarp c;
-  c.lane = lane;
-  c.cw = (warp - 4) >> 2;
-  c.ew = warp - 4;
-  c.row0 = c.cw * 64 + (warp & 3) * 16 + (lane >> 2);
-  c.col0 = 2 * (lane & 3);
-  c.a_off = (uint32_t)c.cw * 64 * 128;
-  const int lrow = (warp & 3) * 16 + (lane & 7) + ((lane >> 3) & 1) * 8;
-  c.a_frag_off = c.a_off + (uint32_t)lrow * 128;
-  c.a_chunk = lane >> 4;
-  c.a_xor = lane & 7;
-  c.wrow0 = c.cw * 64 + (warp & 3) * 16;
-  c.ebuf = smem_u32(smem + Cfg::kStages * Cfg::kStageBytes + 256) + c.ew * (2 * 16 * kEpiCols * 4);
-  c.rbuf = c.ebuf + 16 * kEpiCols * 4;
-  c.rmap = smem_u32(smem + Cfg::kStages * Cfg::kStageBytes + 256 + Cfg::kEpiBufBytes) + c.ew * 16 * 8;
-  return c;
-}
-
-__device__ __forceinline__ void res_issue(const GemmParams& p, const ConsumerWarp& c, const float* res, int n0,
-                                          int half) {
-  const int n = n0 + 4 * (c.lane & 7);
-#pragma unroll
-  for (int k = 0; k < 2; ++k) {
-    const int r = 8 * half + (c.lane >> 3) + 4 * k;
-    const long long m = ld_shared_s64(c.rmap + 8 * r);
-    const uint32_t dst = c.rbuf + (r * kEpiCols + 4 * (c.lane & 7)) * 4;
-    const float* src = res + (m >= 0 ? m * p.ldr + n : 0);
-    if (p.vec_ok) {
-      const int cols = m >= 0 ? min(max(p.N - n, 0), 4) : 0;
-      cp_async_cg16(dst, cols ? src : res, 4 * cols);
-    } else {
-#pragma unroll
-      for (int e = 0; e < 4; ++e) {
-        const bool in = m >= 0 && n + e < p.N;
-        cp_async_ca4(dst + 4 * e, in ? src + e : res, in ? 4 : 0);
-      }
-    }
-  }
-  cp_async_commit();
-}
-
-template <int BN>
-__device__ __forceinline__ void res_prefetch(const GemmParams& p, const ConsumerWarp& c, const float* res, int mt,
-                                             int nt) {
-  if (c.lane < 16) {
-    const RowInfo ri = row_info(p, mt, c.wrow0 + c.lane);
-    st_shared_s64(c.rmap + 8 * c.lane, ri.ok ? ri.mr : -1);
-  }
-  __syncwarp();
-  res_issue(p, c, res, nt * BN, 0);
-  res_issue(p, c, res, nt * BN, 1);
-}
-
-__device__ __forceinline__ void wait_turn(int cw) {
-  if (cw == 0) bar_sync<kTurnBar, 256>(); else bar_sync<kTurnBar + 1, 256>();
-}
-__device__ __forceinline__ void pass_turn(int cw) {
-  if (cw == 0) bar_arrive<kTurnBar + 1, 256>(); else bar_arrive<kTurnBar, 256>();
-}
-
-template <int NSPLIT, int BN>
-__device__ __forceinline__ void mma_piece(const GemmParams& p, const ConsumerWarp& c, uint8_t* smem, uint64_t* full_bar,
-                                          uint64_t* empty_bar, int kbeg, int kend, int& stage, uint32_t& phase,
-                                          float (&acc)[BN / 2], float (&part)[64],
-                                          uint32_t (&afr)[BK / 16][GemmCfg<NSPLIT, BN>::kRegPlanes][4]) {
-  using Cfg = GemmCfg<NSPLIT, BN>;
-  constexpr int kRegPlanes = Cfg::kRegPlanes;
-#pragma unroll
-  for (int i = 0; i < BN / 2; ++i) acc[i] = 0.f;
-  int kb = kbeg % p.num_kb;
-  for (int ki = kbeg; ki < kend; ++ki) {
-    const int nks = (++kb == p.num_kb) ? p.k_last_steps : BK / 16;
-    if (kb == p.num_kb) kb = 0;
-    mbar_wait(&full_bar[stage], phase);
-    const uint32_t sa = smem_u32(smem + stage * Cfg::kStageBytes);
-    const uint32_t a_lo = sa + kTileBytes + c.a_off;
-    const uint32_t b_hi = sa + NSPLIT * kTileBytes, b_lo = b_hi + Cfg::kBTileBytes;
-    {
-      const uint32_t fa = sa + c.a_frag_off;
-#pragma unroll
-      for (int ks = 0; ks < BK / 16; ++ks) {
-        const uint32_t sw = (uint32_t)(((2 * ks + c.a_chunk) ^ c.a_xor) << 4);
-#pragma unroll
-        for (int s = 0; s < kRegPlanes; ++s) ldmatrix_x4(afr[ks][s], fa + s * kTileBytes + sw);
-      }
-    }
-#pragma unroll
-    for (int hn = 0; hn < BN / 128; ++hn) {
-      const uint32_t bo = (uint32_t)hn * 128 * 128;
-      wait_turn(c.cw);
-      wgmma_fence_regs(part);
-      wgmma_fence();
-#pragma unroll
-      for (int ks = 0; ks < BK / 16; ++ks) {
-        if (ks >= nks) break;
-        const uint64_t bdh = gmma_desc_sw128(b_hi + bo + ks * 32);
-        wgmma_rs_n128<0>(part, afr[ks][0], bdh, ks > 0 ? 1 : 0);
-        if (NSPLIT == 2) {
-          wgmma_rs_n128<0>(part, afr[ks][0], gmma_desc_sw128(b_lo + bo + ks * 32), 1);
-          if (kRegPlanes == 2)
-            wgmma_rs_n128<0>(part, afr[ks][1], bdh, 1);
-          else
-            wgmma_ss_n128<0>(part, gmma_desc_sw128(a_lo + ks * 32), bdh, 1);
-        }
-      }
-      wgmma_commit();
-      pass_turn(c.cw);
-      wgmma_wait<0>();
-      wgmma_fence_regs(part);
-#pragma unroll
-      for (int ks = 0; ks < BK / 16; ++ks)
-#pragma unroll
-        for (int s = 0; s < kRegPlanes; ++s) wgmma_fence_regs(afr[ks][s]);
-#pragma unroll
-      for (int i = 0; i < 64; ++i) acc[hn * 64 + i] += part[i];
-    }
-    __syncwarp();
-    if (c.lane == 0) mbar_arrive(&empty_bar[stage]);
-    if (++stage == Cfg::kStages) {
-      stage = 0;
-      phase ^= 1;
-    }
-  }
-}
-
-template <int BN>
-__device__ __forceinline__ void sk_contribute(const GemmParams& p, const ConsumerWarp& c, const float (&acc)[BN / 2]) {
-  float* part = p.sk_part + (size_t)blockIdx.x * BM * 256;
-#pragma unroll
-  for (int i = 0; i < BN / 8; ++i) {
-#pragma unroll
-    for (int h = 0; h < 2; ++h)
-      *reinterpret_cast<float2*>(part + (size_t)(c.row0 + 8 * h) * 256 + 8 * i + c.col0) =
-          make_float2(acc[4 * i + 2 * h], acc[4 * i + 2 * h + 1]);
-  }
-  __threadfence();
-  __syncwarp();
-  if (c.lane == 0) sk_flag_publish(p.sk_flags + blockIdx.x * kEpiWarps + c.ew);
-}
-
-template <int BN>
-__device__ __forceinline__ void sk_collect(const GemmParams& p, const ConsumerWarp& c, const SkSched& sched, int tile,
-                                           int k_iters, float (&acc)[BN / 2]) {
-  const long long tile_kend = (long long)(tile + 1) * k_iters;
-  for (int pp = blockIdx.x + 1; pp < (int)gridDim.x && (long long)pp * sched.W / gridDim.x < tile_kend; ++pp) {
-    unsigned int* flag = p.sk_flags + pp * kEpiWarps + c.ew;
-    if (c.lane == 0) {
-      while (sk_flag_peek(flag) == 0) {
-      }
-    }
-    __syncwarp();
-    __threadfence();
-    const float* part = p.sk_part + (size_t)pp * BM * 256;
-#pragma unroll
-    for (int i = 0; i < BN / 8; ++i) {
-#pragma unroll
-      for (int h = 0; h < 2; ++h) {
-        const float2 a = __ldcg(reinterpret_cast<const float2*>(part + (size_t)(c.row0 + 8 * h) * 256 + 8 * i + c.col0));
-        acc[4 * i + 2 * h] += a.x;
-        acc[4 * i + 2 * h + 1] += a.y;
-      }
-    }
-    __syncwarp();
-    if (c.lane == 0) *reinterpret_cast<volatile unsigned int*>(flag) = 0u;
-  }
-}
-
-__device__ __forceinline__ GemmParams problem_params(const GemmParams& p, const GemmGroup* grp, int g) {
-  GemmParams pg = p;
-  const GroupProblem& gp = grp->prob[g];
-  pg.bias = gp.bias;
-  pg.residual = gp.residual;
-  pg.out_f32 = gp.out_f32;
-  pg.out_hi = gp.out_hi;
-  pg.out_lo = gp.out_lo;
-  return pg;
-}
-
-template <int BN, int ACT, int OUT>
-__device__ __forceinline__ void epilogue_piece(const GemmParams& p, const GemmParams& pq, const ConsumerWarp& cs,
-                                               const float (&acc)[BN / 2], int mt, int nt) {
-  const int lane = cs.lane;
-  const int lr = lane >> 3, c4 = 4 * (lane & 7);
-  long long of_map, ob_map;
-  int rows_ok = 0;
-  {
-    const RowInfo ri = row_info(p, mt, cs.wrow0 + (lane & 15));
-    of_map = ri.mo * pq.ldo_f32;
-    ob_map = ri.mo * pq.ldo_bf;
-#pragma unroll
-    for (int q = 0; q < 4; ++q) rows_ok |= (__shfl_sync(0xffffffffu, (int)ri.ok, 4 * q + lr) & 1) << q;
-  }
-  const uint32_t e_wr = cs.ebuf + ((lane >> 2) * kEpiCols + cs.col0) * 4, e_sw = ((lane >> 2) & 3) * 32;
-  const uint32_t e_rd = cs.ebuf + (lr * kEpiCols + (c4 ^ (lr << 3))) * 4;
-  const uint32_t r_rd = cs.rbuf + (lr * kEpiCols + c4) * 4;
-  constexpr int kChunks = BN / kEpiCols;
-#pragma unroll 1
-  for (int c = 0; c < kChunks; ++c) {
-    const int n0 = nt * BN + c * kEpiCols, n = n0 + c4;
-    const bool full = pq.vec_ok && n + 4 <= pq.N;
-    const float4 b = epilogue_bias4(pq, n, full);
-#pragma unroll
-    for (int cc = 0; cc < kChunks; ++cc) {
-      if (cc != c) continue;
-#pragma unroll
-      for (int j = 0; j < kEpiCols / 8; ++j)
-#pragma unroll
-        for (int h = 0; h < 2; ++h) {
-          const int i = cc * (kEpiCols / 8) + j;
-          st_shared_v2(e_wr + h * 8 * kEpiCols * 4 + ((j * 32) ^ e_sw), acc[4 * i + 2 * h], acc[4 * i + 2 * h + 1]);
-        }
-    }
-    auto store_rows = [&](int half) {
-#pragma unroll 1
-      for (int q = 2 * half; q < 2 * half + 2; ++q) {
-        const float4 v = ld_shared_v4(e_rd + q * 4 * kEpiCols * 4);
-        const float4 rv = pq.residual ? ld_shared_v4(r_rd + q * 4 * kEpiCols * 4) : make_float4(0.f, 0.f, 0.f, 0.f);
-        const long long of = (OUT & kOutF32) ? __shfl_sync(0xffffffffu, of_map, 4 * q + lr) + n : 0;
-        const long long ob = (OUT & kOutSplit) ? __shfl_sync(0xffffffffu, ob_map, 4 * q + lr) + n : 0;
-        if (rows_ok & (1 << q)) epilogue_store4<ACT, OUT>(pq, v, b, rv, of, ob, n, full);
-      }
-    };
-    if (pq.residual) cp_async_wait<1>();
-    __syncwarp();
-    store_rows(0);
-    if (pq.residual) {
-      __syncwarp();
-      if (c + 1 < kChunks) {
-        res_issue(p, cs, pq.residual, n0 + kEpiCols, 0);
-        cp_async_wait<1>();
-      } else {
-        cp_async_wait<0>();
-      }
-      __syncwarp();
-    }
-    store_rows(1);
-    __syncwarp();
-    if (pq.residual && c + 1 < kChunks) res_issue(p, cs, pq.residual, n0 + kEpiCols, 1);
-  }
-}
-
-template <int NSPLIT, int BN, bool GROUPED, bool SK, int ACT, int OUT>
-__device__ __forceinline__ void gemm_tc_body(const CUtensorMap (*maps)[4], const GemmParams& p, const GemmGroup* grp) {
-  static_assert(!SK || (BN == 256 && !GROUPED), "stream-K: single-problem kernel with 256-wide tiles only");
-  using Cfg = GemmCfg<NSPLIT, BN>;
-  constexpr int ST = Cfg::kStages;
-  extern __shared__ uint8_t smem_raw[];
-  uint8_t* smem = reinterpret_cast<uint8_t*>((reinterpret_cast<uintptr_t>(smem_raw) + 1023) &
-                                             ~static_cast<uintptr_t>(1023));
-  uint64_t* full_bar = reinterpret_cast<uint64_t*>(smem + ST * Cfg::kStageBytes);
-  uint64_t* empty_bar = full_bar + ST;
-
-  const int warp = threadIdx.x >> 5;
-  const int tpp = p.tiles_m * p.tiles_n;
-  const int num_tiles = GROUPED ? tpp * grp->count : tpp;
-  const int k_iters = p.taps * p.num_kb;
-  const SkSched sched = sk_schedule<SK>(p, blockIdx.x, gridDim.x, num_tiles, k_iters);
-
-  if (threadIdx.x == 0) {
-    tma_prefetch_desc(&maps[0][0]);
-    tma_prefetch_desc(&maps[0][2]);
-    if (NSPLIT == 2) {
-      tma_prefetch_desc(&maps[0][1]);
-      tma_prefetch_desc(&maps[0][3]);
-    }
-    for (int s = 0; s < ST; ++s) {
-      mbar_init(&full_bar[s], 1);
-      mbar_init(&empty_bar[s], kEpiWarps);
-    }
-    fence_barrier_init();
-  }
-  __syncthreads();
-
-  if (warp < 4) {
-    setmaxnreg_dec<40>();
-    if (warp == 0) produce<NSPLIT, BN, GROUPED>(maps, p, sched, tpp, k_iters, smem, full_bar, empty_bar);
-  } else {
-    setmaxnreg_inc<232>();
-    const ConsumerWarp c = consumer_warp<Cfg>(smem, warp, threadIdx.x & 31);
-    int stage = 0;
-    uint32_t phase = 0;
-    float acc[BN / 2];
-    float part[64];
-    uint32_t afr[BK / 16][Cfg::kRegPlanes][4];
-    if (c.cw == 1) pass_turn(c.cw);
-    for (int si = 0; si < sched.n_seg; ++si) {
-      int tile, kbeg, kend;
-      sk_piece(sched, si, k_iters, tile, kbeg, kend);
-      const PieceCoords pc = piece_coords<GROUPED>(p, tpp, tile);
-      const float* res = GROUPED ? grp->prob[pc.g].residual : p.residual;
-      if (res && !(SK && kbeg > 0) && !(p.debug & 2))
-        res_prefetch<BN>(p, c, res, pc.mt, pc.nt);
-      mma_piece<NSPLIT, BN>(p, c, smem, full_bar, empty_bar, kbeg, kend, stage, phase, acc, part, afr);
-      const bool sk_contrib = SK && kbeg > 0;
-      const bool sk_owner = SK && kbeg == 0 && kend < k_iters;
-      if (SK && sk_contrib) {
-        sk_contribute<BN>(p, c, acc);
-        continue;
-      }
-      if (SK && sk_owner) sk_collect<BN>(p, c, sched, tile, k_iters, acc);
-      if (p.debug & 2) continue;
-      if constexpr (GROUPED)
-        epilogue_piece<BN, ACT, OUT>(p, problem_params(p, grp, pc.g), c, acc, pc.mt, pc.nt);
-      else
-        epilogue_piece<BN, ACT, OUT>(p, p, c, acc, pc.mt, pc.nt);
-    }
-    if (c.cw == 0) wait_turn(c.cw);
-  }
-}
-
-struct GemmMaps1 {
-  CUtensorMap m[1][4];
-};
-
-template <int NSPLIT, int BN, bool SK, int ACT, int OUT>
-__global__ void __launch_bounds__(kGemmThreads, 1)
-gemm_tc_kernel(const __grid_constant__ GemmMaps1 maps, const GemmParams p) {
-  gemm_tc_body<NSPLIT, BN, false, SK, ACT, OUT>(maps.m, p, nullptr);
-}
-
-template <int NSPLIT, int BN, int ACT, int OUT>
-__global__ void __launch_bounds__(kGemmThreads, 1)
-gemm_tc_grouped_kernel(const __grid_constant__ GemmGroupMaps maps, const __grid_constant__ GemmGroup grp,
-                       const GemmParams p) {
-  gemm_tc_body<NSPLIT, BN, true, false, ACT, OUT>(maps.m, p, &grp);
-}
-
-template <typename Cfg, typename Kernel, typename... Args>
-static int launch_kernel(Kernel kernel, bool (&done)[kMaxDevices], const char* what, int grid, cudaStream_t stream,
-                         const Args&... args) {
-  const int dev_ = current_device();
-  if (!done[dev_]) {
-    cudaError_t e = cudaFuncSetAttribute(kernel, cudaFuncAttributeMaxDynamicSharedMemorySize, Cfg::kSmemBytes);
-    if (e != cudaSuccess) return set_error(MTT_ERR_LAUNCH, "%s: cudaFuncSetAttribute: %s", what, cudaGetErrorString(e));
-    done[dev_] = true;
-  }
-  kernel<<<grid, kGemmThreads, Cfg::kSmemBytes, stream>>>(args...);
-  return check_launch(what);
-}
-
-template <int ACT_, int OUT_>
-struct EpiKind {
-  static constexpr int ACT = ACT_, OUT = OUT_;
-};
-template <int ACT, typename F>
-static int with_epilogue_out(const GemmParams& p, F&& f) {
-  if (!p.out_hi) return f(EpiKind<ACT, kOutF32>{});
-  if (!p.out_f32) return f(EpiKind<ACT, kOutSplit>{});
-  return f(EpiKind<ACT, kOutBoth>{});
-}
-template <typename F>
-static int with_epilogue(const GemmParams& p, F&& f) {
-  switch (p.act) {
-    case MTT_ACT_NONE: return with_epilogue_out<MTT_ACT_NONE>(p, f);
-    case MTT_ACT_GELU: return with_epilogue_out<MTT_ACT_GELU>(p, f);
-    case MTT_ACT_RELU: return with_epilogue_out<MTT_ACT_RELU>(p, f);
-  }
-  return set_error(MTT_ERR_BAD_SHAPE, "mtt_gemm: no kernel for act=%d", p.act);
-}
-
-template <typename F>
-static int with_tile(int nsplit, int bn, F&& f) {
-  if (bn == 256) return nsplit == 2 ? f(GemmCfg<2, 256>{}) : f(GemmCfg<1, 256>{});
-  return nsplit == 2 ? f(GemmCfg<2, 128>{}) : f(GemmCfg<1, 128>{});
-}
+static int b_box_rows(int bn) { return bn == 176 ? 88 : bn; }
 
 template <typename Maps>
 static int launch_gemm(const Maps& maps, const GemmGroup* grp, const GemmParams& p, int nsplit, int bn, int grid,
                        cudaStream_t stream) {
-  constexpr bool kGrouped = std::is_same<Maps, GemmGroupMaps>::value;
-  const bool sk = p.sk_tiles > 0;
-  const char* what = kGrouped ? "mtt_gemm_grouped" : sk ? "mtt_gemm(stream-K)" : "mtt_gemm";
-  return with_tile(nsplit, bn, [&](auto cfg) {
-    using Cfg = decltype(cfg);
-    return with_epilogue(p, [&](auto e) {
-      constexpr int NSPLIT = Cfg::kNsplit, BN = Cfg::kBN, ACT = decltype(e)::ACT, OUT = decltype(e)::OUT;
-      static bool done[2][kMaxDevices] = {};
-      if constexpr (kGrouped) {
-        return launch_kernel<Cfg>(gemm_tc_grouped_kernel<NSPLIT, BN, ACT, OUT>, done[0], what, grid, stream, maps, *grp,
-                                  p);
-      } else {
-        if constexpr (BN == 256)
-          if (sk)
-            return launch_kernel<Cfg>(gemm_tc_kernel<NSPLIT, BN, true, ACT, OUT>, done[1], what, grid, stream, maps, p);
-        return launch_kernel<Cfg>(gemm_tc_kernel<NSPLIT, BN, false, ACT, OUT>, done[0], what, grid, stream, maps, p);
-      }
-    });
-  });
+  if (bn == 176) return launch_gemm_176(maps, grp, p, nsplit, grid, stream);
+  if (bn == 256)
+    return nsplit == 2 ? launch_gemm_cfg<GemmCfg<2, 256>>(maps, grp, p, grid, stream)
+                       : launch_gemm_cfg<GemmCfg<1, 256>>(maps, grp, p, grid, stream);
+  return nsplit == 2 ? launch_gemm_cfg<GemmCfg<2, 128>>(maps, grp, p, grid, stream)
+                     : launch_gemm_cfg<GemmCfg<1, 128>>(maps, grp, p, grid, stream);
 }
 
 int launch_gemm_tiles_grouped(const mtt_gemm_desc* d, int count, int bn, cudaStream_t stream) {
@@ -543,7 +24,7 @@
   grp.count = count;
   for (int g = 0; g < count; ++g) {
     GemmParams pg;
-    int rc = gemm_prepare(&d[g], bn, pg, gm.m[g]);
+    int rc = gemm_prepare(&d[g], b_box_rows(bn), pg, gm.m[g]);
     if (rc) return rc;
     pg.tiles_n = (d[g].N + bn - 1) / bn;
     if (g == 0) {
@@ -587,7 +68,7 @@
 int launch_gemm_tiles(const mtt_gemm_desc* d, int bn, cudaStream_t stream) {
   GemmParams p;
   GemmMaps1 gm;
-  int rc = gemm_prepare(d, bn, p, gm.m[0]);
+  int rc = gemm_prepare(d, b_box_rows(bn), p, gm.m[0]);
   if (rc) return rc;
   p.tiles_n = (d->N + bn - 1) / bn;
   const int tiles = p.tiles_m * p.tiles_n;
diff --git a/multi-task-transformer_b200/csrc/gemm_tc176.cu b/multi-task-transformer_b200/csrc/gemm_tc176.cu
--- /dev/null
+++ b/multi-task-transformer_b200/csrc/gemm_tc176.cu
@@ -0,0 +1,15 @@
+#include "gemm_tc_body.cuh"
+
+namespace mtt {
+
+template <typename Maps>
+int launch_gemm_176(const Maps& maps, const GemmGroup* grp, const GemmParams& p, int nsplit, int grid,
+                    cudaStream_t stream) {
+  return nsplit == 2 ? launch_gemm_cfg<GemmCfg<2, 176>>(maps, grp, p, grid, stream)
+                     : launch_gemm_cfg<GemmCfg<1, 176>>(maps, grp, p, grid, stream);
+}
+template int launch_gemm_176<GemmMaps1>(const GemmMaps1&, const GemmGroup*, const GemmParams&, int, int, cudaStream_t);
+template int launch_gemm_176<GemmGroupMaps>(const GemmGroupMaps&, const GemmGroup*, const GemmParams&, int, int,
+                                            cudaStream_t);
+
+}
diff --git a/multi-task-transformer_b200/csrc/gemm_tc_body.cuh b/multi-task-transformer_b200/csrc/gemm_tc_body.cuh
--- /dev/null
+++ b/multi-task-transformer_b200/csrc/gemm_tc_body.cuh
@@ -0,0 +1,695 @@
+#pragma once
+#include <type_traits>
+
+#include "gemm_common.cuh"
+
+namespace mtt {
+
+constexpr int kEpiCols = 32;
+
+template <int NSPLIT, int BN>
+struct GemmCfg {
+  static_assert(BN == 128 || BN == 176 || BN == 256, "tile widths: 128, 176, 256");
+  static constexpr int kNsplit = NSPLIT, kBN = BN;
+  static constexpr uint32_t kBTileBytes = BN * BK * 2;
+  static constexpr uint32_t kStageBytes = NSPLIT * (kTileBytes + kBTileBytes);
+  static constexpr int kStages = (200 * 1024) / kStageBytes;
+  static constexpr int kHalfN = BN == 176 ? 88 : 128;
+  static constexpr int kASlots = NSPLIT == 2 ? 3 : 6, kBSlots = NSPLIT == 2 ? 4 : 8;
+  static constexpr uint32_t kBHalfBytes = kHalfN * BK * 2;
+  static constexpr uint32_t kRingBytes =
+      BN == 176 ? kASlots * NSPLIT * kTileBytes + kBSlots * NSPLIT * kBHalfBytes : kStages * kStageBytes;
+  static constexpr int kBars = BN == 176 ? kASlots + kBSlots : kStages;
+  static constexpr int kRingPeriod = 4 * kASlots;
+  static constexpr uint32_t kEpiBufBytes = kEpiWarps * 2 * 16 * kEpiCols * 4;
+  static constexpr uint32_t kRowMapBytes = kEpiWarps * 16 * 8;
+  static constexpr uint32_t kSmemBytes = kRingBytes + 256 + kEpiBufBytes + kRowMapBytes + 1024;
+  static_assert(kSmemBytes <= 227 * 1024, "exceeds the per-block shared memory of sm_90");
+  static constexpr int kRegPlanes = BN == 256 ? 1 : NSPLIT;
+};
+
+struct SkSched {
+  int n_sk;
+  int tile0, k0_0, k1_0;
+  int k1_1;
+  int dp_first, dp_step;
+  int n_seg;
+  long long W;
+};
+template <bool SK>
+__host__ __device__ __forceinline__ SkSched sk_schedule(const GemmParams& p, int pair, int num_pairs, int num_tiles, int k_iters) {
+  SkSched s;
+  s.n_sk = 0;
+  s.tile0 = s.k0_0 = s.k1_0 = s.k1_1 = 0;
+  s.W = 0;
+  s.dp_first = pair;
+  s.dp_step = num_pairs;
+  if (SK && p.sk_tiles > 0) {
+    s.W = (long long)p.sk_tiles * k_iters;
+    const long long b = (long long)pair * s.W / num_pairs, e = (long long)(pair + 1) * s.W / num_pairs;
+    if (e > b) {
+      const int t0 = (int)(b / k_iters);
+      const long long t0_end = (long long)(t0 + 1) * k_iters;
+      s.tile0 = t0;
+      s.k0_0 = (int)(b - (long long)t0 * k_iters);
+      s.k1_0 = (int)((e < t0_end ? e : t0_end) - (long long)t0 * k_iters);
+      s.n_sk = 1;
+      if (e > t0_end) {
+        s.k1_1 = (int)(e - t0_end);
+        s.n_sk = 2;
+      }
+    }
+    s.dp_first = p.sk_tiles + pair;
+  }
+  const int left = num_tiles - s.dp_first;
+  s.n_seg = s.n_sk + (left > 0 ? (left + s.dp_step - 1) / s.dp_step : 0);
+  return s;
+}
+__host__ __device__ __forceinline__ void sk_piece(const SkSched& s, int si, int k_iters, int& tile, int& k0, int& k1) {
+  if (si < s.n_sk) {
+    tile = s.tile0 + si;
+    k0 = si == 0 ? s.k0_0 : 0;
+    k1 = si == 0 ? s.k1_0 : s.k1_1;
+  } else {
+    tile = s.dp_first + (si - s.n_sk) * s.dp_step;
+    k0 = 0;
+    k1 = k_iters;
+  }
+}
+__device__ __forceinline__ void sk_flag_publish(unsigned int* f) {
+  asm volatile("st.release.gpu.global.u32 [%0], %1;" ::"l"(f), "r"(1u) : "memory");
+}
+__device__ __forceinline__ unsigned int sk_flag_peek(const unsigned int* f) {
+  unsigned int v;
+  asm volatile("ld.acquire.gpu.global.u32 %0, [%1];" : "=r"(v) : "l"(f) : "memory");
+  return v;
+}
+
+
+constexpr uint32_t kTurnBar = 1;
+
+struct PieceCoords {
+  int g, mt, nt;
+};
+template <bool GROUPED>
+__device__ __forceinline__ PieceCoords piece_coords(const GemmParams& p, int tpp, int tile) {
+  const int g = GROUPED ? tile / tpp : 0;
+  const int tl = GROUPED ? tile - g * tpp : tile;
+  return PieceCoords{g, tl % p.tiles_m, tl / p.tiles_m};
+}
+
+template <int NSPLIT, int BN, bool GROUPED>
+__device__ __forceinline__ void produce(const CUtensorMap (*maps)[4], const GemmParams& p, const SkSched& sched,
+                                        int tpp, int k_iters, uint8_t* smem, uint64_t* full_bar, uint64_t* empty_bar) {
+  using Cfg = GemmCfg<NSPLIT, BN>;
+  int stage = 0;
+  uint32_t phase = 0;
+  const uint32_t stage_tx = NSPLIT * (p.a_box_bytes + Cfg::kBTileBytes);
+  for (int si = 0; si < sched.n_seg; ++si) {
+    int tile, kbeg, kend;
+    sk_piece(sched, si, k_iters, tile, kbeg, kend);
+    const PieceCoords pc = piece_coords<GROUPED>(p, tpp, tile);
+    const CUtensorMap* tmA_hi = &maps[pc.g][0];
+    const CUtensorMap* tmA_lo = &maps[pc.g][1];
+    const CUtensorMap* tmB_hi = &maps[pc.g][2];
+    const CUtensorMap* tmB_lo = &maps[pc.g][3];
+    for (int ki = kbeg; ki < kend; ++ki) {
+      const int tap = ki / p.num_kb, kb = ki - tap * p.num_kb;
+      const int dy = (tap / p.ksize - p.ksize / 2) * p.dil;
+      const int dx = (tap % p.ksize - p.ksize / 2) * p.dil;
+      mbar_wait(&empty_bar[stage], phase ^ 1);
+      uint8_t* sa = smem + stage * Cfg::kStageBytes;
+      uint8_t* sb = sa + NSPLIT * kTileBytes;
+      if (elect_one()) {
+        if (p.debug & 1) {
+          mbar_arrive(&full_bar[stage]);
+        } else {
+          mbar_arrive_expect_tx(&full_bar[stage], stage_tx);
+          load_a_tile<NSPLIT>(p, tmA_hi, tmA_lo, sa, &full_bar[stage], pc.mt, kb, dy, dx);
+          const int kcoord = tap * p.cin_pad + kb * BK;
+          tma_load_2d(sb, tmB_hi, &full_bar[stage], kcoord, pc.nt * BN);
+          if (NSPLIT == 2) tma_load_2d(sb + Cfg::kBTileBytes, tmB_lo, &full_bar[stage], kcoord, pc.nt * BN);
+        }
+      }
+      __syncwarp();
+      if (++stage == Cfg::kStages) {
+        stage = 0;
+        phase ^= 1;
+      }
+    }
+  }
+}
+
+template <int NSPLIT, int BN, bool GROUPED>
+__device__ __forceinline__ void produce_rings(const CUtensorMap (*maps)[4], const GemmParams& p, const SkSched& sched,
+                                              int tpp, int k_iters, uint8_t* smem, uint64_t* full_bar,
+                                              uint64_t* empty_bar) {
+  using Cfg = GemmCfg<NSPLIT, BN>;
+  constexpr int NA = Cfg::kASlots, NBK = Cfg::kBSlots / 2;
+  uint8_t* sb0 = smem + NA * NSPLIT * kTileBytes;
+  int cnt = 0;
+  for (int si = 0; si < sched.n_seg; ++si) {
+    int tile, kbeg, kend;
+    sk_piece(sched, si, k_iters, tile, kbeg, kend);
+    const PieceCoords pc = piece_coords<GROUPED>(p, tpp, tile);
+    const CUtensorMap* tmA_hi = &maps[pc.g][0];
+    const CUtensorMap* tmA_lo = &maps[pc.g][1];
+    const CUtensorMap* tmB_hi = &maps[pc.g][2];
+    const CUtensorMap* tmB_lo = &maps[pc.g][3];
+    for (int ki = kbeg; ki < kend; ++ki) {
+      const int tap = ki / p.num_kb, kb = ki - tap * p.num_kb;
+      const int dy = (tap / p.ksize - p.ksize / 2) * p.dil;
+      const int dx = (tap % p.ksize - p.ksize / 2) * p.dil;
+      const int a = cnt % NA, j = cnt % NBK;
+      const uint32_t aph = (cnt / NA) & 1, bph = (cnt / NBK) & 1;
+      mbar_wait(&empty_bar[a], aph ^ 1);
+      if (elect_one()) {
+        if (p.debug & 1) {
+          mbar_arrive(&full_bar[a]);
+        } else {
+          mbar_arrive_expect_tx(&full_bar[a], NSPLIT * p.a_box_bytes);
+          load_a_tile<NSPLIT>(p, tmA_hi, tmA_lo, smem + a * NSPLIT * kTileBytes, &full_bar[a], pc.mt, kb, dy, dx);
+        }
+      }
+      __syncwarp();
+      const int kcoord = tap * p.cin_pad + kb * BK;
+#pragma unroll
+      for (int hn = 0; hn < 2; ++hn) {
+        const int b = 2 * j + hn;
+        uint8_t* sb = sb0 + b * NSPLIT * Cfg::kBHalfBytes;
+        mbar_wait(&empty_bar[NA + b], bph ^ 1);
+        if (elect_one()) {
+          if (p.debug & 1) {
+            mbar_arrive(&full_bar[NA + b]);
+          } else {
+            const int n0 = pc.nt * BN + hn * Cfg::kHalfN;
+            mbar_arrive_expect_tx(&full_bar[NA + b], NSPLIT * Cfg::kBHalfBytes);
+            tma_load_2d(sb, tmB_hi, &full_bar[NA + b], kcoord, n0);
+            if (NSPLIT == 2) tma_load_2d(sb + Cfg::kBHalfBytes, tmB_lo, &full_bar[NA + b], kcoord, n0);
+          }
+        }
+        __syncwarp();
+      }
+      if (++cnt == Cfg::kRingPeriod) cnt = 0;
+    }
+  }
+}
+
+struct ConsumerWarp {
+  int lane;
+  int cw;
+  int ew;
+  int row0, col0;
+  int wrow0;
+  uint32_t a_off;
+  uint32_t a_frag_off;
+  int a_chunk, a_xor;
+  uint32_t ebuf, rbuf, rmap;
+};
+template <typename Cfg>
+__device__ __forceinline__ ConsumerWarp consumer_warp(uint8_t* smem, int warp, int lane) {
+  ConsumerWarp c;
+  c.lane = lane;
+  c.cw = (warp - 4) >> 2;
+  c.ew = warp - 4;
+  c.row0 = c.cw * 64 + (warp & 3) * 16 + (lane >> 2);
+  c.col0 = 2 * (lane & 3);
+  c.a_off = (uint32_t)c.cw * 64 * 128;
+  const int lrow = (warp & 3) * 16 + (lane & 7) + ((lane >> 3) & 1) * 8;
+  c.a_frag_off = c.a_off + (uint32_t)lrow * 128;
+  c.a_chunk = lane >> 4;
+  c.a_xor = lane & 7;
+  c.wrow0 = c.cw * 64 + (warp & 3) * 16;
+  c.ebuf = smem_u32(smem + Cfg::kRingBytes + 256) + c.ew * (2 * 16 * kEpiCols * 4);
+  c.rbuf = c.ebuf + 16 * kEpiCols * 4;
+  c.rmap = smem_u32(smem + Cfg::kRingBytes + 256 + Cfg::kEpiBufBytes) + c.ew * 16 * 8;
+  return c;
+}
+
+__device__ __forceinline__ void res_issue(const GemmParams& p, const ConsumerWarp& c, const float* res, int n0,
+                                          int half) {
+  const int n = n0 + 4 * (c.lane & 7);
+#pragma unroll
+  for (int k = 0; k < 2; ++k) {
+    const int r = 8 * half + (c.lane >> 3) + 4 * k;
+    const long long m = ld_shared_s64(c.rmap + 8 * r);
+    const uint32_t dst = c.rbuf + (r * kEpiCols + 4 * (c.lane & 7)) * 4;
+    const float* src = res + (m >= 0 ? m * p.ldr + n : 0);
+    if (p.vec_ok) {
+      const int cols = m >= 0 ? min(max(p.N - n, 0), 4) : 0;
+      cp_async_cg16(dst, cols ? src : res, 4 * cols);
+    } else {
+#pragma unroll
+      for (int e = 0; e < 4; ++e) {
+        const bool in = m >= 0 && n + e < p.N;
+        cp_async_ca4(dst + 4 * e, in ? src + e : res, in ? 4 : 0);
+      }
+    }
+  }
+  cp_async_commit();
+}
+
+template <int BN>
+__device__ __forceinline__ void res_issue_next(const GemmParams& p, const ConsumerWarp& cs, const float* res, int n0,
+                                               int c, int half) {
+  constexpr int kTail = BN % kEpiCols;
+  if constexpr (kTail != 0) {
+    if (c + 2 == (BN + kEpiCols - 1) / kEpiCols) {
+      GemmParams pt = p;
+      pt.N = min(p.N, n0 + kEpiCols + kTail);
+      res_issue(pt, cs, res, n0 + kEpiCols, half);
+      return;
+    }
+  }
+  res_issue(p, cs, res, n0 + kEpiCols, half);
+}
+
+template <int BN>
+__device__ __forceinline__ void res_prefetch(const GemmParams& p, const ConsumerWarp& c, const float* res, int mt,
+                                             int nt) {
+  if (c.lane < 16) {
+    const RowInfo ri = row_info(p, mt, c.wrow0 + c.lane);
+    st_shared_s64(c.rmap + 8 * c.lane, ri.ok ? ri.mr : -1);
+  }
+  __syncwarp();
+  res_issue(p, c, res, nt * BN, 0);
+  res_issue(p, c, res, nt * BN, 1);
+}
+
+__device__ __forceinline__ void wait_turn(int cw) {
+  if (cw == 0) bar_sync<kTurnBar, 256>(); else bar_sync<kTurnBar + 1, 256>();
+}
+__device__ __forceinline__ void pass_turn(int cw) {
+  if (cw == 0) bar_arrive<kTurnBar + 1, 256>(); else bar_arrive<kTurnBar, 256>();
+}
+
+template <int HN>
+__device__ __forceinline__ void wgmma_rs_half(float (&d)[HN / 2], const uint32_t (&a)[4], uint64_t bdesc, int scale_d) {
+  if constexpr (HN == 88)
+    wgmma_rs_n88<0>(d, a, bdesc, scale_d);
+  else
+    wgmma_rs_n128<0>(d, a, bdesc, scale_d);
+}
+template <int HN>
+__device__ __forceinline__ void wgmma_ss_half(float (&d)[HN / 2], uint64_t adesc, uint64_t bdesc, int scale_d) {
+  if constexpr (HN == 88)
+    wgmma_ss_n88<0>(d, adesc, bdesc, scale_d);
+  else
+    wgmma_ss_n128<0>(d, adesc, bdesc, scale_d);
+}
+
+template <int NSPLIT, int BN>
+__device__ __forceinline__ void mma_piece(const GemmParams& p, const ConsumerWarp& c, uint8_t* smem, uint64_t* full_bar,
+                                          uint64_t* empty_bar, int kbeg, int kend, int& stage, uint32_t& phase,
+                                          float (&acc)[BN / 2], float (&part)[GemmCfg<NSPLIT, BN>::kHalfN / 2],
+                                          uint32_t (&afr)[BK / 16][GemmCfg<NSPLIT, BN>::kRegPlanes][4]) {
+  using Cfg = GemmCfg<NSPLIT, BN>;
+  constexpr int kRegPlanes = Cfg::kRegPlanes;
+  constexpr int HN = Cfg::kHalfN;
+#pragma unroll
+  for (int i = 0; i < BN / 2; ++i) acc[i] = 0.f;
+  int kb = kbeg % p.num_kb;
+  for (int ki = kbeg; ki < kend; ++ki) {
+    const int nks = (++kb == p.num_kb) ? p.k_last_steps : BK / 16;
+    if (kb == p.num_kb) kb = 0;
+    mbar_wait(&full_bar[stage], phase);
+    const uint32_t sa = smem_u32(smem + stage * Cfg::kStageBytes);
+    const uint32_t a_lo = sa + kTileBytes + c.a_off;
+    const uint32_t b_hi = sa + NSPLIT * kTileBytes, b_lo = b_hi + Cfg::kBTileBytes;
+    {
+      const uint32_t fa = sa + c.a_frag_off;
+#pragma unroll
+      for (int ks = 0; ks < BK / 16; ++ks) {
+        const uint32_t sw = (uint32_t)(((2 * ks + c.a_chunk) ^ c.a_xor) << 4);
+#pragma unroll
+        for (int s = 0; s < kRegPlanes; ++s) ldmatrix_x4(afr[ks][s], fa + s * kTileBytes + sw);
+      }
+    }
+#pragma unroll
+    for (int hn = 0; hn < BN / HN; ++hn) {
+      const uint32_t bo = (uint32_t)hn * HN * 128;
+      wait_turn(c.cw);
+      wgmma_fence_regs(part);
+      wgmma_fence();
+#pragma unroll
+      for (int ks = 0; ks < BK / 16; ++ks) {
+        if (ks >= nks) break;
+        const uint64_t bdh = gmma_desc_sw128(b_hi + bo + ks * 32);
+        wgmma_rs_half<HN>(part, afr[ks][0], bdh, ks > 0 ? 1 : 0);
+        if (NSPLIT == 2) {
+          wgmma_rs_half<HN>(part, afr[ks][0], gmma_desc_sw128(b_lo + bo + ks * 32), 1);
+          if (kRegPlanes == 2)
+            wgmma_rs_half<HN>(part, afr[ks][1], bdh, 1);
+          else
+            wgmma_ss_half<HN>(part, gmma_desc_sw128(a_lo + ks * 32), bdh, 1);
+        }
+      }
+      wgmma_commit();
+      pass_turn(c.cw);
+      wgmma_wait<0>();
+      wgmma_fence_regs(part);
+#pragma unroll
+      for (int ks = 0; ks < BK / 16; ++ks)
+#pragma unroll
+        for (int s = 0; s < kRegPlanes; ++s) wgmma_fence_regs(afr[ks][s]);
+#pragma unroll
+      for (int i = 0; i < HN / 2; ++i) acc[hn * (HN / 2) + i] += part[i];
+    }
+    __syncwarp();
+    if (c.lane == 0) mbar_arrive(&empty_bar[stage]);
+    if (++stage == Cfg::kStages) {
+      stage = 0;
+      phase ^= 1;
+    }
+  }
+}
+
+template <int NSPLIT, int BN>
+__device__ __forceinline__ void mma_piece_rings(const GemmParams& p, const ConsumerWarp& c, uint8_t* smem,
+                                                uint64_t* full_bar, uint64_t* empty_bar, int kbeg, int kend, int& cnt,
+                                                float (&acc)[BN / 2], float (&part)[GemmCfg<NSPLIT, BN>::kHalfN / 2],
+                                                uint32_t (&afr)[BK / 16][GemmCfg<NSPLIT, BN>::kRegPlanes][4]) {
+  using Cfg = GemmCfg<NSPLIT, BN>;
+  constexpr int HN = Cfg::kHalfN, NA = Cfg::kASlots, NBK = Cfg::kBSlots / 2;
+  static_assert(Cfg::kRegPlanes == NSPLIT, "the A ring is released before the chains: A must be in registers");
+  const uint32_t sb0 = smem_u32(smem + NA * NSPLIT * kTileBytes);
+#pragma unroll
+  for (int i = 0; i < BN / 2; ++i) acc[i] = 0.f;
+  int kb = kbeg % p.num_kb;
+  for (int ki = kbeg; ki < kend; ++ki) {
+    const int nks = (++kb == p.num_kb) ? p.k_last_steps : BK / 16;
+    if (kb == p.num_kb) kb = 0;
+    const int a = cnt % NA, j = cnt % NBK;
+    const uint32_t aph = (cnt / NA) & 1, bph = (cnt / NBK) & 1;
+    mbar_wait(&full_bar[a], aph);
+    {
+      const uint32_t fa = smem_u32(smem + a * NSPLIT * kTileBytes) + c.a_frag_off;
+#pragma unroll
+      for (int ks = 0; ks < BK / 16; ++ks) {
+        const uint32_t sw = (uint32_t)(((2 * ks + c.a_chunk) ^ c.a_xor) << 4);
+#pragma unroll
+        for (int s = 0; s < NSPLIT; ++s) ldmatrix_x4(afr[ks][s], fa + s * kTileBytes + sw);
+      }
+    }
+    __syncwarp();
+    if (c.lane == 0) mbar_arrive(&empty_bar[a]);
+#pragma unroll
+    for (int hn = 0; hn < 2; ++hn) {
+      const int b = 2 * j + hn;
+      const uint32_t b_hi = sb0 + b * NSPLIT * Cfg::kBHalfBytes, b_lo = b_hi + Cfg::kBHalfBytes;
+      mbar_wait(&full_bar[NA + b], bph);
+      wait_turn(c.cw);
+      wgmma_fence_regs(part);
+      wgmma_fence();
+#pragma unroll
+      for (int ks = 0; ks < BK / 16; ++ks) {
+        if (ks >= nks) break;
+        const uint64_t bdh = gmma_desc_sw128(b_hi + ks * 32);
+        wgmma_rs_half<HN>(part, afr[ks][0], bdh, ks > 0 ? 1 : 0);
+        if (NSPLIT == 2) {
+          wgmma_rs_half<HN>(part, afr[ks][0], gmma_desc_sw128(b_lo + ks * 32), 1);
+          wgmma_rs_half<HN>(part, afr[ks][NSPLIT - 1], bdh, 1);
+        }
+      }
+      wgmma_commit();
+      pass_turn(c.cw);
+      wgmma_wait<0>();
+      wgmma_fence_regs(part);
+#pragma unroll
+      for (int ks = 0; ks < BK / 16; ++ks)
+#pragma unroll
+        for (int s = 0; s < NSPLIT; ++s) wgmma_fence_regs(afr[ks][s]);
+#pragma unroll
+      for (int i = 0; i < HN / 2; ++i) acc[hn * (HN / 2) + i] += part[i];
+      __syncwarp();
+      if (c.lane == 0) mbar_arrive(&empty_bar[NA + b]);
+    }
+    if (++cnt == Cfg::kRingPeriod) cnt = 0;
+  }
+}
+
+template <int BN>
+__device__ __forceinline__ void sk_contribute(const GemmParams& p, const ConsumerWarp& c, const float (&acc)[BN / 2]) {
+  float* part = p.sk_part + (size_t)blockIdx.x * BM * 256;
+#pragma unroll
+  for (int i = 0; i < BN / 8; ++i) {
+#pragma unroll
+    for (int h = 0; h < 2; ++h)
+      *reinterpret_cast<float2*>(part + (size_t)(c.row0 + 8 * h) * 256 + 8 * i + c.col0) =
+          make_float2(acc[4 * i + 2 * h], acc[4 * i + 2 * h + 1]);
+  }
+  __threadfence();
+  __syncwarp();
+  if (c.lane == 0) sk_flag_publish(p.sk_flags + blockIdx.x * kEpiWarps + c.ew);
+}
+
+template <int BN>
+__device__ __forceinline__ void sk_collect(const GemmParams& p, const ConsumerWarp& c, const SkSched& sched, int tile,
+                                           int k_iters, float (&acc)[BN / 2]) {
+  const long long tile_kend = (long long)(tile + 1) * k_iters;
+  for (int pp = blockIdx.x + 1; pp < (int)gridDim.x && (long long)pp * sched.W / gridDim.x < tile_kend; ++pp) {
+    unsigned int* flag = p.sk_flags + pp * kEpiWarps + c.ew;
+    if (c.lane == 0) {
+      while (sk_flag_peek(flag) == 0) {
+      }
+    }
+    __syncwarp();
+    __threadfence();
+    const float* part = p.sk_part + (size_t)pp * BM * 256;
+#pragma unroll
+    for (int i = 0; i < BN / 8; ++i) {
+#pragma unroll
+      for (int h = 0; h < 2; ++h) {
+        const float2 a = __ldcg(reinterpret_cast<const float2*>(part + (size_t)(c.row0 + 8 * h) * 256 + 8 * i + c.col0));
+        acc[4 * i + 2 * h] += a.x;
+        acc[4 * i + 2 * h + 1] += a.y;
+      }
+    }
+    __syncwarp();
+    if (c.lane == 0) *reinterpret_cast<volatile unsigned int*>(flag) = 0u;
+  }
+}
+
+__device__ __forceinline__ GemmParams problem_params(const GemmParams& p, const GemmGroup* grp, int g) {
+  GemmParams pg = p;
+  const GroupProblem& gp = grp->prob[g];
+  pg.bias = gp.bias;
+  pg.residual = gp.residual;
+  pg.out_f32 = gp.out_f32;
+  pg.out_hi = gp.out_hi;
+  pg.out_lo = gp.out_lo;
+  return pg;
+}
+
+template <int BN, int ACT, int OUT>
+__device__ __forceinline__ void epilogue_piece(const GemmParams& p, const GemmParams& pq, const ConsumerWarp& cs,
+                                               const float (&acc)[BN / 2], int mt, int nt) {
+  const int lane = cs.lane;
+  const int lr = lane >> 3, c4 = 4 * (lane & 7);
+  long long of_map, ob_map;
+  int rows_ok = 0;
+  {
+    const RowInfo ri = row_info(p, mt, cs.wrow0 + (lane & 15));
+    of_map = ri.mo * pq.ldo_f32;
+    ob_map = ri.mo * pq.ldo_bf;
+#pragma unroll
+    for (int q = 0; q < 4; ++q) rows_ok |= (__shfl_sync(0xffffffffu, (int)ri.ok, 4 * q + lr) & 1) << q;
+  }
+  const uint32_t e_wr = cs.ebuf + ((lane >> 2) * kEpiCols + cs.col0) * 4, e_sw = ((lane >> 2) & 3) * 32;
+  const uint32_t e_rd = cs.ebuf + (lr * kEpiCols + (c4 ^ (lr << 3))) * 4;
+  const uint32_t r_rd = cs.rbuf + (lr * kEpiCols + c4) * 4;
+  constexpr int kChunks = (BN + kEpiCols - 1) / kEpiCols, kTail = BN % kEpiCols;
+#pragma unroll 1
+  for (int c = 0; c < kChunks; ++c) {
+    const int n0 = nt * BN + c * kEpiCols, n = n0 + c4;
+    const bool full = pq.vec_ok && n + 4 <= pq.N;
+    const float4 b = epilogue_bias4(pq, n, full);
+#pragma unroll
+    for (int cc = 0; cc < kChunks; ++cc) {
+      if (cc != c) continue;
+#pragma unroll
+      for (int j = 0; j < kEpiCols / 8; ++j)
+#pragma unroll
+        for (int h = 0; h < 2; ++h) {
+          const int i = cc * (kEpiCols / 8) + j;
+          if constexpr (kTail != 0)
+            if (i >= BN / 8) continue;
+          st_shared_v2(e_wr + h * 8 * kEpiCols * 4 + ((j * 32) ^ e_sw), acc[4 * i + 2 * h], acc[4 * i + 2 * h + 1]);
+        }
+    }
+    auto store_rows = [&](int half) {
+#pragma unroll 1
+      for (int q = 2 * half; q < 2 * half + 2; ++q) {
+        const float4 v = ld_shared_v4(e_rd + q * 4 * kEpiCols * 4);
+        const float4 rv = pq.residual ? ld_shared_v4(r_rd + q * 4 * kEpiCols * 4) : make_float4(0.f, 0.f, 0.f, 0.f);
+        const long long of = (OUT & kOutF32) ? __shfl_sync(0xffffffffu, of_map, 4 * q + lr) + n : 0;
+        const long long ob = (OUT & kOutSplit) ? __shfl_sync(0xffffffffu, ob_map, 4 * q + lr) + n : 0;
+        if constexpr (kTail != 0)
+          if (c + 1 == kChunks && c4 >= kTail) continue;
+        if (rows_ok & (1 << q)) epilogue_store4<ACT, OUT>(pq, v, b, rv, of, ob, n, full);
+      }
+    };
+    if (pq.residual) cp_async_wait<1>();
+    __syncwarp();
+    store_rows(0);
+    if (pq.residual) {
+      __syncwarp();
+      if (c + 1 < kChunks) {
+        res_issue_next<BN>(p, cs, pq.residual, n0, c, 0);
+        cp_async_wait<1>();
+      } else {
+        cp_async_wait<0>();
+      }
+      __syncwarp();
+    }
+    store_rows(1);
+    __syncwarp();
+    if (pq.residual && c + 1 < kChunks) res_issue_next<BN>(p, cs, pq.residual, n0, c, 1);
+  }
+}
+
+template <int NSPLIT, int BN, bool GROUPED, bool SK, int ACT, int OUT>
+__device__ __forceinline__ void gemm_tc_body(const CUtensorMap (*maps)[4], const GemmParams& p, const GemmGroup* grp) {
+  static_assert(!SK || (BN == 256 && !GROUPED), "stream-K: single-problem kernel with 256-wide tiles only");
+  using Cfg = GemmCfg<NSPLIT, BN>;
+  constexpr int ST = Cfg::kBars;
+  extern __shared__ uint8_t smem_raw[];
+  uint8_t* smem = reinterpret_cast<uint8_t*>((reinterpret_cast<uintptr_t>(smem_raw) + 1023) &
+                                             ~static_cast<uintptr_t>(1023));
+  uint64_t* full_bar = reinterpret_cast<uint64_t*>(smem + Cfg::kRingBytes);
+  uint64_t* empty_bar = full_bar + ST;
+
+  const int warp = threadIdx.x >> 5;
+  const int tpp = p.tiles_m * p.tiles_n;
+  const int num_tiles = GROUPED ? tpp * grp->count : tpp;
+  const int k_iters = p.taps * p.num_kb;
+  const SkSched sched = sk_schedule<SK>(p, blockIdx.x, gridDim.x, num_tiles, k_iters);
+
+  if (threadIdx.x == 0) {
+    tma_prefetch_desc(&maps[0][0]);
+    tma_prefetch_desc(&maps[0][2]);
+    if (NSPLIT == 2) {
+      tma_prefetch_desc(&maps[0][1]);
+      tma_prefetch_desc(&maps[0][3]);
+    }
+    for (int s = 0; s < ST; ++s) {
+      mbar_init(&full_bar[s], 1);
+      mbar_init(&empty_bar[s], kEpiWarps);
+    }
+    fence_barrier_init();
+  }
+  __syncthreads();
+
+  if (warp < 4) {
+    setmaxnreg_dec<40>();
+    if (warp == 0) {
+      if constexpr (BN == 176)
+        produce_rings<NSPLIT, BN, GROUPED>(maps, p, sched, tpp, k_iters, smem, full_bar, empty_bar);
+      else
+        produce<NSPLIT, BN, GROUPED>(maps, p, sched, tpp, k_iters, smem, full_bar, empty_bar);
+    }
+  } else {
+    setmaxnreg_inc<232>();
+    const ConsumerWarp c = consumer_warp<Cfg>(smem, warp, threadIdx.x & 31);
+    int stage = 0;
+    uint32_t phase = 0;
+    float acc[BN / 2];
+    float part[Cfg::kHalfN / 2];
+    uint32_t afr[BK / 16][Cfg::kRegPlanes][4];
+    if (c.cw == 1) pass_turn(c.cw);
+    for (int si = 0; si < sched.n_seg; ++si) {
+      int tile, kbeg, kend;
+      sk_piece(sched, si, k_iters, tile, kbeg, kend);
+      const PieceCoords pc = piece_coords<GROUPED>(p, tpp, tile);
+      const float* res = GROUPED ? grp->prob[pc.g].residual : p.residual;
+      if (res && !(SK && kbeg > 0) && !(p.debug & 2))
+        res_prefetch<BN>(p, c, res, pc.mt, pc.nt);
+      if constexpr (BN == 176)
+        mma_piece_rings<NSPLIT, BN>(p, c, smem, full_bar, empty_bar, kbeg, kend, stage, acc, part, afr);
+      else
+        mma_piece<NSPLIT, BN>(p, c, smem, full_bar, empty_bar, kbeg, kend, stage, phase, acc, part, afr);
+      const bool sk_contrib = SK && kbeg > 0;
+      const bool sk_owner = SK && kbeg == 0 && kend < k_iters;
+      if (SK && sk_contrib) {
+        sk_contribute<BN>(p, c, acc);
+        continue;
+      }
+      if (SK && sk_owner) sk_collect<BN>(p, c, sched, tile, k_iters, acc);
+      if (p.debug & 2) continue;
+      if constexpr (GROUPED)
+        epilogue_piece<BN, ACT, OUT>(p, problem_params(p, grp, pc.g), c, acc, pc.mt, pc.nt);
+      else
+        epilogue_piece<BN, ACT, OUT>(p, p, c, acc, pc.mt, pc.nt);
+    }
+    if (c.cw == 0) wait_turn(c.cw);
+  }
+}
+
+template <int NSPLIT, int BN, bool SK, int ACT, int OUT>
+__global__ void __launch_bounds__(kGemmThreads, 1)
+gemm_tc_kernel(const __grid_constant__ GemmMaps1 maps, const GemmParams p) {
+  gemm_tc_body<NSPLIT, BN, false, SK, ACT, OUT>(maps.m, p, nullptr);
+}
+
+template <int NSPLIT, int BN, int ACT, int OUT>
+__global__ void __launch_bounds__(kGemmThreads, 1)
+gemm_tc_grouped_kernel(const __grid_constant__ GemmGroupMaps maps, const __grid_constant__ GemmGroup grp,
+                       const GemmParams p) {
+  gemm_tc_body<NSPLIT, BN, true, false, ACT, OUT>(maps.m, p, &grp);
+}
+
+template <typename Cfg, typename Kernel, typename... Args>
+static int launch_kernel(Kernel kernel, bool (&done)[kMaxDevices], const char* what, int grid, cudaStream_t stream,
+                         const Args&... args) {
+  const int dev_ = current_device();
+  if (!done[dev_]) {
+    cudaError_t e = cudaFuncSetAttribute(kernel, cudaFuncAttributeMaxDynamicSharedMemorySize, Cfg::kSmemBytes);
+    if (e != cudaSuccess) return set_error(MTT_ERR_LAUNCH, "%s: cudaFuncSetAttribute: %s", what, cudaGetErrorString(e));
+    done[dev_] = true;
+  }
+  kernel<<<grid, kGemmThreads, Cfg::kSmemBytes, stream>>>(args...);
+  return check_launch(what);
+}
+
+template <int ACT_, int OUT_>
+struct EpiKind {
+  static constexpr int ACT = ACT_, OUT = OUT_;
+};
+template <int ACT, typename F>
+static int with_epilogue_out(const GemmParams& p, F&& f) {
+  if (!p.out_hi) return f(EpiKind<ACT, kOutF32>{});
+  if (!p.out_f32) return f(EpiKind<ACT, kOutSplit>{});
+  return f(EpiKind<ACT, kOutBoth>{});
+}
+template <typename F>
+static int with_epilogue(const GemmParams& p, F&& f) {
+  switch (p.act) {
+    case MTT_ACT_NONE: return with_epilogue_out<MTT_ACT_NONE>(p, f);
+    case MTT_ACT_GELU: return with_epilogue_out<MTT_ACT_GELU>(p, f);
+    case MTT_ACT_RELU: return with_epilogue_out<MTT_ACT_RELU>(p, f);
+  }
+  return set_error(MTT_ERR_BAD_SHAPE, "mtt_gemm: no kernel for act=%d", p.act);
+}
+
+template <typename Cfg, typename Maps>
+static int launch_gemm_cfg(const Maps& maps, const GemmGroup* grp, const GemmParams& p, int grid, cudaStream_t stream) {
+  constexpr bool kGrouped = std::is_same<Maps, GemmGroupMaps>::value;
+  constexpr int NSPLIT = Cfg::kNsplit, BN = Cfg::kBN;
+  const bool sk = p.sk_tiles > 0;
+  const char* what = kGrouped ? "mtt_gemm_grouped" : sk ? "mtt_gemm(stream-K)" : "mtt_gemm";
+  return with_epilogue(p, [&](auto e) {
+    constexpr int ACT = decltype(e)::ACT, OUT = decltype(e)::OUT;
+    static bool done[2][kMaxDevices] = {};
+    if constexpr (kGrouped) {
+      return launch_kernel<Cfg>(gemm_tc_grouped_kernel<NSPLIT, BN, ACT, OUT>, done[0], what, grid, stream, maps, *grp,
+                                p);
+    } else {
+      if constexpr (BN == 256)
+        if (sk)
+          return launch_kernel<Cfg>(gemm_tc_kernel<NSPLIT, BN, true, ACT, OUT>, done[1], what, grid, stream, maps, p);
+      return launch_kernel<Cfg>(gemm_tc_kernel<NSPLIT, BN, false, ACT, OUT>, done[0], what, grid, stream, maps, p);
+    }
+  });
+}
+
+}
diff --git a/multi-task-transformer_b200/csrc/ptx.cuh b/multi-task-transformer_b200/csrc/ptx.cuh
--- a/multi-task-transformer_b200/csrc/ptx.cuh
+++ b/multi-task-transformer_b200/csrc/ptx.cuh
@@ -202,6 +202,15 @@
 }
 
 template <int kTransB>
+__device__ __forceinline__ void wgmma_ss_n88(float (&d)[44], uint64_t adesc, uint64_t bdesc, int scale_d) {
+  asm volatile(
+      "{\n\t.reg .pred p;\n\tsetp.ne.b32 p, %46, 0;\n\t"
+      "wgmma.mma_async.sync.aligned.m64n88k16.f32.bf16.bf16 {%0, %1, %2, %3, %4, %5, %6, %7, %8, %9, %10, %11, %12, %13, %14, %15, %16, %17, %18, %19, %20, %21, %22, %23, %24, %25, %26, %27, %28, %29, %30, %31, %32, %33, %34, %35, %36, %37, %38, %39, %40, %41, %42, %43}, %44, %45, p, 1, 1, 0, %47;\n\t}\n"
+      : "+f"(d[0]), "+f"(d[1]), "+f"(d[2]), "+f"(d[3]), "+f"(d[4]), "+f"(d[5]), "+f"(d[6]), "+f"(d[7]), "+f"(d[8]), "+f"(d[9]), "+f"(d[10]), "+f"(d[11]), "+f"(d[12]), "+f"(d[13]), "+f"(d[14]), "+f"(d[15]), "+f"(d[16]), "+f"(d[17]), "+f"(d[18]), "+f"(d[19]), "+f"(d[20]), "+f"(d[21]), "+f"(d[22]), "+f"(d[23]), "+f"(d[24]), "+f"(d[25]), "+f"(d[26]), "+f"(d[27]), "+f"(d[28]), "+f"(d[29]), "+f"(d[30]), "+f"(d[31]), "+f"(d[32]), "+f"(d[33]), "+f"(d[34]), "+f"(d[35]), "+f"(d[36]), "+f"(d[37]), "+f"(d[38]), "+f"(d[39]), "+f"(d[40]), "+f"(d[41]), "+f"(d[42]), "+f"(d[43])
+      : "l"(adesc), "l"(bdesc), "r"(scale_d), "n"(kTransB));
+}
+
+template <int kTransB>
 __device__ __forceinline__ void wgmma_ss_n128(float (&d)[64], uint64_t adesc, uint64_t bdesc, int scale_d) {
   asm volatile(
       "{\n\t.reg .pred p;\n\tsetp.ne.b32 p, %66, 0;\n\t"
@@ -225,6 +234,15 @@
       "{\n\t.reg .pred p;\n\tsetp.ne.b32 p, %37, 0;\n\t"
       "wgmma.mma_async.sync.aligned.m64n64k16.f32.bf16.bf16 {%0, %1, %2, %3, %4, %5, %6, %7, %8, %9, %10, %11, %12, %13, %14, %15, %16, %17, %18, %19, %20, %21, %22, %23, %24, %25, %26, %27, %28, %29, %30, %31}, {%32, %33, %34, %35}, %36, p, 1, 1, %38;\n\t}\n"
       : "+f"(d[0]), "+f"(d[1]), "+f"(d[2]), "+f"(d[3]), "+f"(d[4]), "+f"(d[5]), "+f"(d[6]), "+f"(d[7]), "+f"(d[8]), "+f"(d[9]), "+f"(d[10]), "+f"(d[11]), "+f"(d[12]), "+f"(d[13]), "+f"(d[14]), "+f"(d[15]), "+f"(d[16]), "+f"(d[17]), "+f"(d[18]), "+f"(d[19]), "+f"(d[20]), "+f"(d[21]), "+f"(d[22]), "+f"(d[23]), "+f"(d[24]), "+f"(d[25]), "+f"(d[26]), "+f"(d[27]), "+f"(d[28]), "+f"(d[29]), "+f"(d[30]), "+f"(d[31])
+      : "r"(a[0]), "r"(a[1]), "r"(a[2]), "r"(a[3]), "l"(bdesc), "r"(scale_d), "n"(kTransB));
+}
+
+template <int kTransB>
+__device__ __forceinline__ void wgmma_rs_n88(float (&d)[44], const uint32_t (&a)[4], uint64_t bdesc, int scale_d) {
+  asm volatile(
+      "{\n\t.reg .pred p;\n\tsetp.ne.b32 p, %49, 0;\n\t"
+      "wgmma.mma_async.sync.aligned.m64n88k16.f32.bf16.bf16 {%0, %1, %2, %3, %4, %5, %6, %7, %8, %9, %10, %11, %12, %13, %14, %15, %16, %17, %18, %19, %20, %21, %22, %23, %24, %25, %26, %27, %28, %29, %30, %31, %32, %33, %34, %35, %36, %37, %38, %39, %40, %41, %42, %43}, {%44, %45, %46, %47}, %48, p, 1, 1, %50;\n\t}\n"
+      : "+f"(d[0]), "+f"(d[1]), "+f"(d[2]), "+f"(d[3]), "+f"(d[4]), "+f"(d[5]), "+f"(d[6]), "+f"(d[7]), "+f"(d[8]), "+f"(d[9]), "+f"(d[10]), "+f"(d[11]), "+f"(d[12]), "+f"(d[13]), "+f"(d[14]), "+f"(d[15]), "+f"(d[16]), "+f"(d[17]), "+f"(d[18]), "+f"(d[19]), "+f"(d[20]), "+f"(d[21]), "+f"(d[22]), "+f"(d[23]), "+f"(d[24]), "+f"(d[25]), "+f"(d[26]), "+f"(d[27]), "+f"(d[28]), "+f"(d[29]), "+f"(d[30]), "+f"(d[31]), "+f"(d[32]), "+f"(d[33]), "+f"(d[34]), "+f"(d[35]), "+f"(d[36]), "+f"(d[37]), "+f"(d[38]), "+f"(d[39]), "+f"(d[40]), "+f"(d[41]), "+f"(d[42]), "+f"(d[43])
       : "r"(a[0]), "r"(a[1]), "r"(a[2]), "r"(a[3]), "l"(bdesc), "r"(scale_d), "n"(kTransB));
 }
 
```

After: 174.2, median of 6. 1.01x the previous value.
